# Siyou-Li/u2Tokenizer

Measured on NVIDIA H100. Metric: ct_volumes_per_sec, higher is better.
Workload: dtype bf16

## Files before the change

### include/u2b200.h

```cpp
#ifndef U2B200_H_
#define U2B200_H_

#include <stdint.h>

#if defined(__GNUC__)
#define U2_API __attribute__((visibility("default")))
#else
#define U2_API
#endif

#ifdef __cplusplus
extern "C" {
#endif

#define U2_OK 0
#define U2_ERR_ARG (-1)
#define U2_ERR_CUDA (-2)
#define U2_ERR_UNSUPPORTED (-3)

#define U2_DT_BF16 0
#define U2_DT_F32 1

#define U2_ACT_NONE 0
#define U2_ACT_GELU 1
#define U2_ACT_SILU 2

#define U2_EPI_NONE 0
#define U2_EPI_EXP_ROW 1
#define U2_EPI_DS_ROW 2

U2_API int u2_version(void);
U2_API const char* u2_last_error(void);
U2_API int u2_device_sm_count(void);

typedef struct u2_gemm_desc {
  int32_t M, N, K;
  int32_t zi, zo;
  int32_t b_zi_div;
  int64_t lda, a_stride_zi, a_stride_zo;
  int64_t ldb, b_stride_zi, b_stride_zo;
  int64_t ldc, c_stride_zi, c_stride_zo;
  int32_t c_dtype;
  float alpha;
  const float* bias;
  int32_t act;
  const void* residual;
  int64_t ldr;
  int32_t res_row_mod;
  int32_t row_div, row_stride, row_off;
  int32_t block_n;
  int32_t a_mn, b_mn;
  int32_t epi_op;
  const float* rowvec;
  int64_t rv_stride_zi, rv_stride_zo;
  const void* mul;
} u2_gemm_desc;

U2_API int u2_gemm_bf16(const void* A, const void* B, void* C, const u2_gemm_desc* desc, void* stream);

U2_API int u2_layernorm_bf16(const void* x, const void* residual, const float* gamma, const float* beta,
                             void* y, void* sum_out, int64_t rows, int32_t E, int64_t ldx, int64_t ldr,
                             int64_t ldy, float eps, void* stream);
U2_API int u2_rmsnorm_bf16(const void* x, const void* residual, const float* gamma, void* y, void* sum_out,
                           int64_t rows, int32_t E, int64_t ldx, int64_t ldr, int64_t ldy, float eps,
                           void* stream);

typedef struct u2_softmax_desc {
  int64_t in_s0, in_s1, in_s2;
  int64_t out_s0, out_s1, out_s2;
  int32_t n0, H, S, n;
  float scale;
  const float* rel_bias;
  int32_t rel_max;
  int32_t causal, causal_off;
  int32_t zero_pad_to;
  int32_t window;
} u2_softmax_desc;
U2_API int u2_softmax_f32_bf16(const float* in, void* out, const u2_softmax_desc* desc, void* stream);

U2_API int u2_silu_mul_bf16(const void* gate_up, void* out, int64_t rows, int32_t I, int64_t ldg,
                            int64_t ldo, int32_t interleaved, void* stream);

U2_API int u2_patchify_f32_bf16(const float* vol, void* rows, int64_t frames, int32_t d0, int32_t d1,
                                int32_t d2, int32_t p0, int32_t p1, int32_t p2, void* stream);
U2_API int u2_patch_embed_f32_bf16(const float* vol, const void* W, const float* bias, const void* pos, void* out,
                                   int64_t frames, int32_t d0, int32_t d1, int32_t d2, int32_t p0, int32_t p1, int32_t p2,
                                   int32_t N, int64_t out_frame_rows, void* stream);
U2_API int u2_set_rows_bf16(void* dst, const void* vec, int64_t n_rows, int64_t row_stride, int64_t row_off,
                            int32_t E, void* stream);
U2_API int u2_vit_frame_rows_bf16(void* dst, const void* cls, int64_t frames, int32_t Sp, int32_t S, int32_t E,
                                  void* stream);
U2_API int u2_transpose_heads_bf16(const void* in, void* out, int32_t B, int32_t S, int32_t H, int32_t Dh,
                                   int64_t in_sb, int64_t in_ss, int64_t in_sh, int64_t out_sb,
                                   int64_t out_sh, int64_t ld_out, void* stream);
U2_API int u2_spp_pool_bf16(const void* x, void* out, int64_t frames, int32_t g0, int32_t g1, int32_t g2,
                            int32_t ps, int32_t E, int64_t in_frame_stride, int64_t in_off, int64_t ldx,
                            int32_t sequence, void* stream);
U2_API int u2_multiscale_pool_bf16(const void* x, void* out, const float* gate_w, float gate_bias,
                                   float* logits_ws, int32_t B, int32_t K, int32_t E, int32_t dynamic,
                                   void* stream);
U2_API int64_t u2_multiscale_pool_ws_elems(int32_t B, int32_t K);
U2_API int u2_embed_splice_bf16(const int64_t* ids, const void* table, const void* vis, void* out, int32_t B,
                                int32_t L, int32_t E, int32_t n_vis, int64_t vocab, void* stream);

U2_API int u2_temporal_attention_bf16(const void* qkv, void* out, int32_t B, int32_t C, int32_t N, int32_t H,
                                      int32_t dh, int64_t ld_qkv, int64_t ld_out, float scale,
                                      const float* rel_bias, int32_t rel_max, void* stream);

typedef struct u2_rope_desc {
  int64_t rows, ld;
  int32_t dh, n_q_heads, n_k_heads, n_v_heads;
  const float* q_norm_w;
  const float* k_norm_w;
  float eps;
  const float* inv_freq;
  int32_t pos0, pos_div, pos_mod;
  const int32_t* pos0_dev;
  void* k_cache;
  void* v_cache;
  int32_t Tmax, rows_per_batch;
  int32_t pos0_per_batch;
} u2_rope_desc;
U2_API int u2_rope_bf16(void* x, const u2_rope_desc* desc, void* stream);

U2_API int u2_decode_attention_bf16(const void* q, const void* k_cache, const void* v_cache, void* out,
                                    int32_t B, int32_t Hq, int32_t Hkv, int32_t dh, int32_t Tmax, int32_t T,
                                    const int32_t* T_dev, int64_t ldq, int64_t ldo, float scale, int32_t T_per_seq,
                                    const int32_t* kv_src, int64_t ld_kv_src, void* stream);
U2_API int u2_decode_attention_window_bf16(const void* q, const void* k_cache, const void* v_cache, void* out,
                                           int32_t B, int32_t Hq, int32_t Hkv, int32_t dh, int32_t Tmax, int32_t T,
                                           const int32_t* T_dev, int64_t ldq, int64_t ldo, float scale,
                                           int32_t T_per_seq, const int32_t* kv_src, int64_t ld_kv_src,
                                           int32_t window, void* stream);

typedef struct u2_gemv_desc {
  int32_t B, N, K;
  int64_t ldx, ldw, ldy, ldr;
  int32_t y_dtype;
  const void* residual;
  const float* norm_gamma;
  float norm_eps;
  int32_t silu_pair;
} u2_gemv_desc;
U2_API int u2_gemv_bf16(const void* x, const void* w, void* y, const u2_gemv_desc* desc, void* stream);
U2_API int u2_argmax_f32(const float* logits, int64_t* out, uint64_t* scratch, int32_t B, int32_t V, int64_t ld,
                         void* stream);

#define U2_DLIN_STREAMK128 0
#define U2_DLIN_TILES64 1
typedef struct u2_dlinear_desc {
  int32_t B, N, K;
  int64_t ldx, ldw, ldy, ldr, ldxg;
  int32_t y_dtype;
  float* ws;
  int32_t* counters;
  const float* ssq_in;
  float eps;
  const void* residual;
  int32_t silu_pair;
  const float* gamma_next;
  void* xg;
  float* ssq_out;
  float* ssq_zero;
  int32_t pdl;
  void* dbg;
  int64_t ws_elems;
  const int32_t* dep_flags;
  int32_t dep_shift;
  int32_t* out_flags;
  int32_t sched;
} u2_dlinear_desc;
U2_API int u2_dlinear_bf16(const void* x, const void* w, void* y, const u2_dlinear_desc* desc, void* stream);
U2_API int64_t u2_dlinear_ws_elems(int32_t N, int32_t K);
typedef struct u2_dlinear_next {
  int32_t pre_stages;
  int32_t lookahead_units;
  int32_t n;
  const void* w[2];
  int32_t N[2], K[2];
  int64_t ldw[2];
  int32_t units[2];
} u2_dlinear_next;
U2_API int u2_dlinear_multi_bf16(const void* const* x, const void* const* w, void* const* y,
                                 const u2_dlinear_desc* descs, int32_t n_ops, uint32_t* gridbar,
                                 const int32_t* step_dev, int32_t pdl, const u2_dlinear_next* next, void* stream);
U2_API int u2_decode_embed_bf16(const int64_t* ids, const void* table, const float* gamma, void* x, void* xg,
                                float* ssq, float* ssq_zero, int32_t* step_counter, int32_t B, int32_t E,
                                int64_t vocab, void* stream);

typedef struct u2_fused_decode_desc {
  int32_t B, Hq, Hkv, dh, Tmax, pos;
  const int32_t* pos_dev;
  int64_t ldq, ldo;
  const float* q_norm_w;
  const float* k_norm_w;
  float eps;
  const float* inv_freq;
  float scale;
  int32_t kv_splits;
  int32_t pdl;
  int32_t pos_per_seq;
  const int32_t* kv_src;
  int64_t ld_kv_src;
  int32_t window;
} u2_fused_decode_desc;
U2_API int u2_decode_attention_fused_bf16(const void* qkv, void* k_cache, void* v_cache, void* out,
                                          const u2_fused_decode_desc* desc, void* stream);

U2_API int u2_topk_rows_f32(const float* scores, int64_t* out_idx, int32_t rows, int32_t T, int32_t K, int64_t ld,
                            int64_t idx_offset_per_row, void* stream);

typedef struct u2_fa_desc {
  int32_t B, H, Sq, Sk, dh;
  float scale;
  int64_t q_sb, q_ss, q_sh;
  int64_t k_sb, k_ss, k_sh;
  int64_t v_sb, v_ss, v_sh;
  int64_t out_sb, out_ss;
  float* lse;
} u2_fa_desc;
U2_API int u2_flash_attention_d64_bf16(const void* q, const void* k, const void* v, void* out, const u2_fa_desc* desc,
                                       void* stream);

U2_API int u2_sample_f32(const float* logits, int64_t* out, int32_t B, int32_t V, int64_t ld, float temperature,
                         int32_t top_k, float top_p, uint64_t seed, const int32_t* step_dev, int32_t step,
                         void* stream);

typedef struct u2_sample_params {
  float temperature;
  int32_t top_k;
  float top_p;
  int32_t reserved;
  uint64_t seed;
} u2_sample_params;
U2_API int u2_sample_dev_f32(const float* logits, int64_t* out, int32_t B, int32_t V, int64_t ld,
                             const u2_sample_params* params_dev, const int32_t* step_dev, int32_t step, void* stream);

#define U2_LP_MAX_EOS 8
#define U2_LP_MAX_BAD_WORDS 256
#define U2_LP_MAX_BAD_TOKENS 2048
typedef struct u2_logits_proc_params {
  float penalty;
  float inv_penalty;
  int32_t ngram;
  int32_t min_new;
  int32_t n_eos;
  int32_t n_bad;
  int32_t eos[U2_LP_MAX_EOS];
  int32_t bad_off[U2_LP_MAX_BAD_WORDS + 1];
  int32_t bad_tok[U2_LP_MAX_BAD_TOKENS];
} u2_logits_proc_params;
U2_API int u2_logits_process_f32(float* logits, int32_t B, int32_t V, int64_t ld, const int64_t* ids, int32_t* hist,
                                 int64_t ld_hist, int32_t hist_cap, const u2_logits_proc_params* params_dev,
                                 const int32_t* step_dev, int32_t step, void* stream);

#define U2_BEAM_MAX_BEAMS 16
#define U2_BEAM_MAX_EOS 8
#define U2_BEAM_MAX_KEEP 144
typedef struct u2_beam_params {
  double length_penalty;
  int32_t num_beams;
  int32_t beams_to_keep;
  int32_t early_stopping;
  int32_t max_new_tokens;
  int32_t n_eos;
  int32_t reserved;
  int32_t eos[U2_BEAM_MAX_EOS];
} u2_beam_params;
typedef struct u2_beam_step_desc {
  const u2_beam_params* params;
  int32_t prompts, V;
  const float* cand_val;
  const int32_t* cand_tok;
  float* running;
  float* fin_score;
  int32_t* fin_info;
  int32_t* flags;
  int64_t* ids;
  int32_t* rec;
  int64_t ld_rec;
  int32_t rec_rows;
  int32_t* kv_src;
  int64_t ld_kv_src;
  const int32_t* pos_dev;
  int32_t* hist;
  int64_t ld_hist;
  int32_t hist_cap;
  const int32_t* step_dev;
} u2_beam_step_desc;
U2_API int u2_log_softmax_f32(const float* x, float* y, int32_t rows, int32_t V, int64_t ldx, int64_t ldy, void* stream);
U2_API int u2_beam_topk_f32(const float* logprobs, int64_t ld, int32_t rows, int32_t V, const float* running,
                            const int32_t* flags, const u2_beam_params* params_dev, float* cand_val, int32_t* cand_tok,
                            void* stream);
U2_API int u2_beam_step(const u2_beam_step_desc* desc, int32_t step, void* stream);

typedef struct u2_logprob_desc {
  int32_t R, V, E;
  int64_t ldh, ldw;
  const int64_t* labels;
  void* ws;
  int64_t ws_bytes;
  float* lse;
  float* logit_sum;
  float* nll_acc;
} u2_logprob_desc;
U2_API int64_t u2_logprob_ws_bytes(int32_t R, int32_t V);
U2_API int u2_lmhead_logprob_bf16(const void* hidden, const void* W, float* logp, const u2_logprob_desc* desc,
                                  void* stream);

#define U2_PP_OK 0
#define U2_PP_EMPTY_FOREGROUND 1
#define U2_PP_DEGENERATE_SHAPE 2
#define U2_PP_FLAT_INTENSITY 3
typedef struct u2_preprocess_info {
  double a_min, a_max;
  int32_t lo[3], hi[3];
  int32_t out[3];
  float sigma[3];
  int32_t tail[3];
  int32_t status;
} u2_preprocess_info;
typedef struct u2_preprocess_desc {
  int32_t D, H, W;
  int32_t target, pad_depth;
  double lower_pct, upper_pct;
  void* ws;
  int64_t ws_bytes;
} u2_preprocess_desc;
U2_API int64_t u2_preprocess_ws_bytes(int32_t D, int32_t H, int32_t W);
U2_API int u2_preprocess_volume_f32(const float* vol, float* out, u2_preprocess_info* info,
                                    const u2_preprocess_desc* desc, void* stream);

#ifdef __cplusplus
}
#endif
#endif
```

### u2tokenizer_b200/_lib.py

```python
from __future__ import annotations

import ctypes as C
from pathlib import Path

_LIB_PATH = Path(__file__).resolve().parent / "libu2b200.so"
_lib = None


class GemmDesc(C.Structure):
    _fields_ = [
        ("M", C.c_int32), ("N", C.c_int32), ("K", C.c_int32),
        ("zi", C.c_int32), ("zo", C.c_int32), ("b_zi_div", C.c_int32),
        ("lda", C.c_int64), ("a_stride_zi", C.c_int64), ("a_stride_zo", C.c_int64),
        ("ldb", C.c_int64), ("b_stride_zi", C.c_int64), ("b_stride_zo", C.c_int64),
        ("ldc", C.c_int64), ("c_stride_zi", C.c_int64), ("c_stride_zo", C.c_int64),
        ("c_dtype", C.c_int32), ("alpha", C.c_float),
        ("bias", C.c_void_p),
        ("act", C.c_int32),
        ("residual", C.c_void_p),
        ("ldr", C.c_int64),
        ("res_row_mod", C.c_int32),
        ("row_div", C.c_int32), ("row_stride", C.c_int32), ("row_off", C.c_int32),
        ("block_n", C.c_int32),
        ("a_mn", C.c_int32), ("b_mn", C.c_int32),
        ("epi_op", C.c_int32),
        ("rowvec", C.c_void_p),
        ("rv_stride_zi", C.c_int64), ("rv_stride_zo", C.c_int64),
        ("mul", C.c_void_p),
    ]


class SoftmaxDesc(C.Structure):
    _fields_ = [
        ("in_s0", C.c_int64), ("in_s1", C.c_int64), ("in_s2", C.c_int64),
        ("out_s0", C.c_int64), ("out_s1", C.c_int64), ("out_s2", C.c_int64),
        ("n0", C.c_int32), ("H", C.c_int32), ("S", C.c_int32), ("n", C.c_int32),
        ("scale", C.c_float),
        ("rel_bias", C.c_void_p),
        ("rel_max", C.c_int32),
        ("causal", C.c_int32), ("causal_off", C.c_int32),
        ("zero_pad_to", C.c_int32),
        ("window", C.c_int32),
    ]


class RopeDesc(C.Structure):
    _fields_ = [
        ("rows", C.c_int64), ("ld", C.c_int64),
        ("dh", C.c_int32), ("n_q_heads", C.c_int32), ("n_k_heads", C.c_int32), ("n_v_heads", C.c_int32),
        ("q_norm_w", C.c_void_p), ("k_norm_w", C.c_void_p),
        ("eps", C.c_float),
        ("inv_freq", C.c_void_p),
        ("pos0", C.c_int32), ("pos_div", C.c_int32), ("pos_mod", C.c_int32),
        ("pos0_dev", C.c_void_p),
        ("k_cache", C.c_void_p), ("v_cache", C.c_void_p),
        ("Tmax", C.c_int32), ("rows_per_batch", C.c_int32),
        ("pos0_per_batch", C.c_int32),
    ]


class GemvDesc(C.Structure):
    _fields_ = [
        ("B", C.c_int32), ("N", C.c_int32), ("K", C.c_int32),
        ("ldx", C.c_int64), ("ldw", C.c_int64), ("ldy", C.c_int64), ("ldr", C.c_int64),
        ("y_dtype", C.c_int32),
        ("residual", C.c_void_p),
        ("norm_gamma", C.c_void_p),
        ("norm_eps", C.c_float),
        ("silu_pair", C.c_int32),
    ]


class DlinearDesc(C.Structure):
    _fields_ = [
        ("B", C.c_int32), ("N", C.c_int32), ("K", C.c_int32),
        ("ldx", C.c_int64), ("ldw", C.c_int64), ("ldy", C.c_int64), ("ldr", C.c_int64), ("ldxg", C.c_int64),
        ("y_dtype", C.c_int32),
        ("ws", C.c_void_p), ("counters", C.c_void_p),
        ("ssq_in", C.c_void_p),
        ("eps", C.c_float),
        ("residual", C.c_void_p),
        ("silu_pair", C.c_int32),
        ("gamma_next", C.c_void_p),
        ("xg", C.c_void_p),
        ("ssq_out", C.c_void_p),
        ("ssq_zero", C.c_void_p),
        ("pdl", C.c_int32),
        ("dbg", C.c_void_p),
        ("ws_elems", C.c_int64),
        ("dep_flags", C.c_void_p), ("dep_shift", C.c_int32), ("out_flags", C.c_void_p),
        ("sched", C.c_int32),
    ]


class FusedDecodeDesc(C.Structure):
    _fields_ = [
        ("B", C.c_int32), ("Hq", C.c_int32), ("Hkv", C.c_int32), ("dh", C.c_int32), ("Tmax", C.c_int32),
        ("pos", C.c_int32),
        ("pos_dev", C.c_void_p),
        ("ldq", C.c_int64), ("ldo", C.c_int64),
        ("q_norm_w", C.c_void_p), ("k_norm_w", C.c_void_p),
        ("eps", C.c_float),
        ("inv_freq", C.c_void_p),
        ("scale", C.c_float),
        ("kv_splits", C.c_int32), ("pdl", C.c_int32),
        ("pos_per_seq", C.c_int32),
        ("kv_src", C.c_void_p), ("ld_kv_src", C.c_int64),
        ("window", C.c_int32),
    ]


class DlinearNext(C.Structure):
    _fields_ = [
        ("pre_stages", C.c_int32), ("lookahead_units", C.c_int32), ("n", C.c_int32),
        ("w", C.c_void_p * 2),
        ("N", C.c_int32 * 2), ("K", C.c_int32 * 2),
        ("ldw", C.c_int64 * 2),
        ("units", C.c_int32 * 2),
    ]


class FaDesc(C.Structure):
    _fields_ = [
        ("B", C.c_int32), ("H", C.c_int32), ("Sq", C.c_int32), ("Sk", C.c_int32), ("dh", C.c_int32),
        ("scale", C.c_float),
        ("q_sb", C.c_int64), ("q_ss", C.c_int64), ("q_sh", C.c_int64),
        ("k_sb", C.c_int64), ("k_ss", C.c_int64), ("k_sh", C.c_int64),
        ("v_sb", C.c_int64), ("v_ss", C.c_int64), ("v_sh", C.c_int64),
        ("out_sb", C.c_int64), ("out_ss", C.c_int64),
        ("lse", C.c_void_p),
    ]


class LogprobDesc(C.Structure):
    _fields_ = [
        ("R", C.c_int32), ("V", C.c_int32), ("E", C.c_int32),
        ("ldh", C.c_int64), ("ldw", C.c_int64),
        ("labels", C.c_void_p), ("ws", C.c_void_p), ("ws_bytes", C.c_int64),
        ("lse", C.c_void_p), ("logit_sum", C.c_void_p), ("nll_acc", C.c_void_p),
    ]


class PreprocessInfo(C.Structure):
    _fields_ = [
        ("a_min", C.c_double), ("a_max", C.c_double),
        ("lo", C.c_int32 * 3), ("hi", C.c_int32 * 3), ("out", C.c_int32 * 3),
        ("sigma", C.c_float * 3), ("tail", C.c_int32 * 3), ("status", C.c_int32),
    ]


class PreprocessDesc(C.Structure):
    _fields_ = [
        ("D", C.c_int32), ("H", C.c_int32), ("W", C.c_int32), ("target", C.c_int32), ("pad_depth", C.c_int32),
        ("lower_pct", C.c_double), ("upper_pct", C.c_double),
        ("ws", C.c_void_p), ("ws_bytes", C.c_int64),
    ]


class SoftmaxBwdDesc(C.Structure):
    _fields_ = [
        ("p_s0", C.c_int64), ("p_s1", C.c_int64), ("p_s2", C.c_int64),
        ("dp_s0", C.c_int64), ("dp_s1", C.c_int64), ("dp_s2", C.c_int64),
        ("ds_s0", C.c_int64), ("ds_s1", C.c_int64), ("ds_s2", C.c_int64),
        ("n0", C.c_int32), ("H", C.c_int32), ("S", C.c_int32), ("n", C.c_int32),
        ("zero_pad_to", C.c_int32),
    ]


class AdamWDesc(C.Structure):
    _fields_ = [
        ("lr", C.c_float), ("beta1", C.c_float), ("beta2", C.c_float), ("eps", C.c_float), ("weight_decay", C.c_float),
        ("step", C.c_int32),
        ("grad_scale", C.c_void_p),
        ("seed", C.c_uint64), ("index_offset", C.c_int64),
    ]


class LoraDesc(C.Structure):
    _fields_ = [
        ("M", C.c_int32), ("K", C.c_int32), ("r", C.c_int32), ("n_adapters", C.c_int32),
        ("ldx", C.c_int64), ("ldu", C.c_int64),
        ("scale", C.c_float), ("p", C.c_float),
        ("seed", C.c_uint64),
        ("stream", C.c_int32 * 3),
        ("accumulate", C.c_int32),
    ]


LP_MAX_EOS, LP_MAX_BAD_WORDS, LP_MAX_BAD_TOKENS = 8, 256, 2048


class LogitsProcParams(C.Structure):
    _fields_ = [
        ("penalty", C.c_float), ("inv_penalty", C.c_float), ("ngram", C.c_int32), ("min_new", C.c_int32),
        ("n_eos", C.c_int32), ("n_bad", C.c_int32),
        ("eos", C.c_int32 * LP_MAX_EOS),
        ("bad_off", C.c_int32 * (LP_MAX_BAD_WORDS + 1)),
        ("bad_tok", C.c_int32 * LP_MAX_BAD_TOKENS),
    ]


BEAM_MAX_BEAMS, BEAM_MAX_EOS, BEAM_MAX_KEEP = 16, 8, 144


class BeamParams(C.Structure):
    _fields_ = [
        ("length_penalty", C.c_double),
        ("num_beams", C.c_int32), ("beams_to_keep", C.c_int32), ("early_stopping", C.c_int32),
        ("max_new_tokens", C.c_int32), ("n_eos", C.c_int32), ("reserved", C.c_int32),
        ("eos", C.c_int32 * BEAM_MAX_EOS),
    ]


class BeamStepDesc(C.Structure):
    _fields_ = [
        ("params", C.c_void_p),
        ("prompts", C.c_int32), ("V", C.c_int32),
        ("cand_val", C.c_void_p), ("cand_tok", C.c_void_p),
        ("running", C.c_void_p), ("fin_score", C.c_void_p), ("fin_info", C.c_void_p), ("flags", C.c_void_p),
        ("ids", C.c_void_p),
        ("rec", C.c_void_p), ("ld_rec", C.c_int64), ("rec_rows", C.c_int32),
        ("kv_src", C.c_void_p), ("ld_kv_src", C.c_int64),
        ("pos_dev", C.c_void_p),
        ("hist", C.c_void_p), ("ld_hist", C.c_int64), ("hist_cap", C.c_int32),
        ("step_dev", C.c_void_p),
    ]


_P, _I, _L, _F = C.c_void_p, C.c_int32, C.c_int64, C.c_float
SIGNATURES = {
    "u2_version": (C.c_int, []),
    "u2_last_error": (C.c_char_p, []),
    "u2_device_sm_count": (C.c_int, []),
    "u2_gemm_bf16": (C.c_int, [_P, _P, _P, C.POINTER(GemmDesc), _P]),
    "u2_layernorm_bf16": (C.c_int, [_P, _P, _P, _P, _P, _P, _L, _I, _L, _L, _L, _F, _P]),
    "u2_rmsnorm_bf16": (C.c_int, [_P, _P, _P, _P, _P, _L, _I, _L, _L, _L, _F, _P]),
    "u2_softmax_f32_bf16": (C.c_int, [_P, _P, C.POINTER(SoftmaxDesc), _P]),
    "u2_silu_mul_bf16": (C.c_int, [_P, _P, _L, _I, _L, _L, _I, _P]),
    "u2_patchify_f32_bf16": (C.c_int, [_P, _P, _L, _I, _I, _I, _I, _I, _I, _P]),
    "u2_patch_embed_f32_bf16": (C.c_int, [_P, _P, _P, _P, _P, _L, _I, _I, _I, _I, _I, _I, _I, _L, _P]),
    "u2_set_rows_bf16": (C.c_int, [_P, _P, _L, _L, _L, _I, _P]),
    "u2_vit_frame_rows_bf16": (C.c_int, [_P, _P, _L, _I, _I, _I, _P]),
    "u2_transpose_heads_bf16": (C.c_int, [_P, _P, _I, _I, _I, _I, _L, _L, _L, _L, _L, _L, _P]),
    "u2_spp_pool_bf16": (C.c_int, [_P, _P, _L, _I, _I, _I, _I, _I, _L, _L, _L, _I, _P]),
    "u2_multiscale_pool_bf16": (C.c_int, [_P, _P, _P, _F, _P, _I, _I, _I, _I, _P]),
    "u2_multiscale_pool_ws_elems": (C.c_int64, [_I, _I]),
    "u2_embed_splice_bf16": (C.c_int, [_P, _P, _P, _P, _I, _I, _I, _I, _L, _P]),
    "u2_temporal_attention_bf16": (C.c_int, [_P, _P, _I, _I, _I, _I, _I, _L, _L, _F, _P, _I, _P]),
    "u2_rope_bf16": (C.c_int, [_P, C.POINTER(RopeDesc), _P]),
    "u2_decode_attention_bf16": (C.c_int, [_P, _P, _P, _P, _I, _I, _I, _I, _I, _I, _P, _L, _L, _F, _I, _P, _L, _P]),
    "u2_decode_attention_window_bf16": (C.c_int, [_P, _P, _P, _P, _I, _I, _I, _I, _I, _I, _P, _L, _L, _F, _I, _P, _L,
                                                  _I, _P]),
    "u2_gemv_bf16": (C.c_int, [_P, _P, _P, C.POINTER(GemvDesc), _P]),
    "u2_argmax_f32": (C.c_int, [_P, _P, _P, _I, _I, _L, _P]),
    "u2_dlinear_bf16": (C.c_int, [_P, _P, _P, C.POINTER(DlinearDesc), _P]),
    "u2_decode_attention_fused_bf16": (C.c_int, [_P, _P, _P, _P, C.POINTER(FusedDecodeDesc), _P]),
    "u2_decode_embed_bf16": (C.c_int, [_P, _P, _P, _P, _P, _P, _P, _P, _I, _I, _L, _P]),
    "u2_flash_attention_d64_bf16": (C.c_int, [_P, _P, _P, _P, C.POINTER(FaDesc), _P]),
    "u2_sample_f32": (C.c_int, [_P, _P, _I, _I, _L, _F, _I, _F, C.c_uint64, _P, _I, _P]),
    "u2_sample_dev_f32": (C.c_int, [_P, _P, _I, _I, _L, _P, _P, _I, _P]),
    "u2_logits_process_f32": (C.c_int, [_P, _I, _I, _L, _P, _P, _L, _I, _P, _P, _I, _P]),
    "u2_topk_rows_f32": (C.c_int, [_P, _P, _I, _I, _I, _L, _L, _P]),
    "u2_log_softmax_f32": (C.c_int, [_P, _P, _I, _I, _L, _L, _P]),
    "u2_beam_topk_f32": (C.c_int, [_P, _L, _I, _I, _P, _P, _P, _P, _P, _P]),
    "u2_beam_step": (C.c_int, [C.POINTER(BeamStepDesc), _I, _P]),
    "u2_dlinear_ws_elems": (C.c_int64, [_I, _I]),
    "u2_dlinear_multi_bf16": (C.c_int, [_P, _P, _P, _P, _I, _P, _P, _I, _P, _P]),
    "u2_preprocess_ws_bytes": (C.c_int64, [_I, _I, _I]),
    "u2_preprocess_volume_f32": (C.c_int, [_P, _P, _P, C.POINTER(PreprocessDesc), _P]),
    "u2_logprob_ws_bytes": (C.c_int64, [_I, _I]),
    "u2_lmhead_logprob_bf16": (C.c_int, [_P, _P, _P, C.POINTER(LogprobDesc), _P]),
    "u2_transpose_bf16": (C.c_int, [_P, _P, _I, _I, _L, _L, _I, _L, _L, _P]),
    "u2_colsum_bf16": (C.c_int, [_P, _P, _L, _L, _L, _P]),
    "u2_gelu_bf16": (C.c_int, [_P, _P, _L, _P]),
    "u2_gelu_bwd_bf16": (C.c_int, [_P, _P, _P, _L, _P]),
    "u2_silu_mul_bwd_bf16": (C.c_int, [_P, _P, _P, _L, _I, _L, _L, _P]),
    "u2_layernorm_bwd_bf16": (C.c_int, [_P, _P, _P, _P, _P, _P, _P, _L, _I, _L, _L, _L, _L, _F, _P]),
    "u2_rmsnorm_bwd_bf16": (C.c_int, [_P, _P, _P, _P, _P, _P, _L, _I, _L, _L, _L, _L, _F, _P]),
    "u2_softmax_bwd_bf16": (C.c_int, [_P, _P, _P, C.POINTER(SoftmaxBwdDesc), _P]),
    "u2_relbias_grad_bf16": (C.c_int, [_P, _P, _I, _I, _I, _I, _L, _L, _L, _I, _P]),
    "u2_rowdot_bf16": (C.c_int, [_P, _P, _P, _I, _I, _I, _I, _L, _L, _L, _L, _L, _L, _P]),
    "u2_temporal_attention_bwd_bf16": (C.c_int, [_P, _P, _P, _I, _I, _I, _I, _I, _L, _L, _L, _F, _P, _P, _I, _P]),
    "u2_rope_bwd_bf16": (C.c_int, [_P, _P, C.POINTER(RopeDesc), _P, _P, _P]),
    "u2_spp_pool_bwd_bf16": (C.c_int, [_P, _P, _L, _I, _I, _I, _I, _I, _L, _L, _L, _L, _I, _P]),
    "u2_multiscale_pool_bwd_bf16": (C.c_int, [_P, _P, _P, _P, _P, _P, _P, _I, _I, _I, _I, _P]),
    "u2_embed_scatter_add_bf16": (C.c_int, [_P, _P, _P, _P, _I, _I, _I, _I, _L, _P]),
    "u2_group_sum_bf16": (C.c_int, [_P, _P, _L, _I, _I, _I, _L, _L, _P]),
    "u2_ce_bwd_f32_bf16": (C.c_int, [_P, _P, _P, _P, _P, _L, _I, _L, _L, _P]),
    "u2_dpo_loss_f32": (C.c_int, [_P, _P, _P, _P, _P, _I, _I, _F, _P]),
    "u2_adamw_bf16": (C.c_int, [_P, _P, _P, _P, _P, _L, C.POINTER(AdamWDesc), _P]),
    "u2_adamw_bf16_mom16": (C.c_int, [_P, _P, _P, _P, _P, _L, C.POINTER(AdamWDesc), _P]),
    "u2_adamw_f32grad": (C.c_int, [_P, _P, _P, _P, _P, _P, _L, C.POINTER(AdamWDesc), _P]),
    "u2_sumsq_bf16": (C.c_int, [_P, _P, _L, _P]),
    "u2_sumsq_f32": (C.c_int, [_P, _P, _L, _P]),
    "u2_add_bf16": (C.c_int, [_P, _P, _L, _P]),
    "u2_cast_f32_bf16": (C.c_int, [_P, _P, _L, _P]),
    "u2_cast_bf16_f32": (C.c_int, [_P, _P, _L, _P]),
    "u2_lora_down_bf16": (C.c_int, [_P, _P, _P, C.POINTER(LoraDesc), _P]),
    "u2_lora_wgrad_bf16": (C.c_int, [_P, _P, _P, C.POINTER(LoraDesc), _P]),
    "u2_lora_dgrad_bf16": (C.c_int, [_P, _P, _P, C.POINTER(LoraDesc), _P]),
}


def lib_path() -> Path:
    return _LIB_PATH


def load():
    global _lib
    if _lib is not None:
        return _lib
    if not _LIB_PATH.exists():
        raise RuntimeError(
            f"{_LIB_PATH} is missing: build it with `python -m u2tokenizer_b200.build` "
            "(there is no CPU / PyTorch fallback for the hot path)")
    lib = C.CDLL(str(_LIB_PATH))
    for name, (res, args) in SIGNATURES.items():
        fn = getattr(lib, name)
        fn.restype = res
        fn.argtypes = args
    _lib = lib
    return lib


KERNELS_PER_CALL = {"u2_multiscale_pool_bf16": 3, "u2_argmax_f32": 2, "u2_lmhead_logprob_bf16": 2,
                    "u2_preprocess_volume_f32": 14, "u2_multiscale_pool_bwd_bf16": 2}
_launches = 0


def launches() -> int:
    return _launches


def add_launches(n: int) -> None:
    global _launches
    _launches += n


def check(rc: int, what: str) -> None:
    global _launches
    _launches += KERNELS_PER_CALL.get(what, 1)
    if rc != 0:
        msg = load().u2_last_error()
        raise RuntimeError(f"{what} failed (code {rc}): {msg.decode() if msg else '?'}")
```

### u2tokenizer_b200/csrc/dlinear_wgmma.cu

```cuda
#include <cuda_bf16.h>
#include <math.h>
#include <stdio.h>
#include <stdlib.h>

#include "host_util.h"
#include "ptx.cuh"
#include "u2b200.h"

namespace u2 {

constexpr int kDlN = 16;
constexpr int kDlK = 64;
constexpr int kDlBBytes = kDlN * kDlK * 2;
constexpr int kDlThreads = 384;
constexpr int kDlMmaWarp0 = 8;
constexpr int kDlAccLd = 20;

template <int kM>
struct DlCfg {
  static constexpr int kABytes = kM * kDlK * 2;
  static constexpr int kStageBytes = kABytes + kDlBBytes;
#ifndef U2_DL_STAGES128
#define U2_DL_STAGES128 10
#endif
  static constexpr int kStages = (kM == 128) ? U2_DL_STAGES128 : 18;
  static constexpr int kAccBytes = 2 * kM * kDlAccLd * 4;
  static constexpr int kSmem = kStages * kStageBytes + kAccBytes + 1024 + 512;
};

struct DlinArgs {
  int B, N, K;
  int num_tiles, kblocks;
  float* ws;
  int max_slots;
  int* counters;
  const float* ssq_in;
  float inv_norm_dim, eps;
  const __nv_bfloat16* residual;
  long long ldr;
  void* y;
  long long ldy;
  int y_dtype;
  int silu_pair;
  const float* gamma_next;
  __nv_bfloat16* xg;
  long long ldxg;
  float* ssq_out;
  float* ssq_part;
  int* ssq_ticket;
  float* ssq_zero;
  const int* dep_flags;
  int dep_shift;
  int* out_flags;
  unsigned long long* dbg;
};

constexpr int kDlMaxOps = 4;

struct DlinMulti {
  CUtensorMap tw[kDlMaxOps];
  CUtensorMap tx[kDlMaxOps];
  DlinArgs op[kDlMaxOps];
  int n_ops;
  unsigned int* gridbar;
  const int* step_dev;
  unsigned long long* dbg;
  CUtensorMap tnext[2];
  int next_tiles[2], next_kblocks[2], next_units[2];
  int n_next;
  int pre_stages;
  int lookahead_units;
};

#define U2_STAMP(op, i)                                                                  \
  do {                                                                                   \
    if (mp.dbg) {                                                                        \
      unsigned long long t__;                                                            \
      asm volatile("mov.u64 %0, %%globaltimer;" : "=l"(t__));                           \
      mp.dbg[(blockIdx.x * kDlMaxOps + (op)) * 8 + (i)] = t__;                           \
    }                                                                                    \
  } while (0)

__device__ __forceinline__ unsigned int ld_acquire_u32(const unsigned int* p) {
  unsigned int v;
  asm volatile("ld.acquire.gpu.global.u32 %0, [%1];" : "=r"(v) : "l"(p) : "memory");
  return v;
}

__device__ __forceinline__ float4 ld_relaxed_f4(const float4* p) {
  float4 v;
  asm volatile("ld.relaxed.gpu.global.v4.f32 {%0, %1, %2, %3}, [%4];"
               : "=f"(v.x), "=f"(v.y), "=f"(v.z), "=f"(v.w)
               : "l"(p)
               : "memory");
  return v;
}

__device__ __forceinline__ void grid_barrier_wait(const unsigned int* bar, unsigned int target) {
  unsigned int v, spins = 0;
  do {
    asm volatile("ld.relaxed.gpu.global.u32 %0, [%1];" : "=r"(v) : "l"(bar) : "memory");
    if (++spins == (1u << 24)) {
      printf("u2 dlinear: grid barrier timed out (CTA %d sees %u of %u arrivals): CTAs of the launch are not co-resident\n",
             (int)blockIdx.x, v, target);
      __trap();
    }
  } while (v < target);
  asm volatile("fence.acq_rel.gpu;" ::: "memory");
}

struct UnitIter {
  int tile, kb, kblocks, tile_step;
  int left;
  __device__ __forceinline__ void next() {
    if (++kb == kblocks) {
      kb = 0;
      tile += tile_step;
    }
    --left;
  }
  __device__ __forceinline__ int seg_len() const {
    const int r = kblocks - kb;
    return r < left ? r : left;
  }
};

__device__ __forceinline__ UnitIter make_iter(int num_tiles, int kblocks, bool tiles) {
  UnitIter it;
  it.kblocks = kblocks;
  if (tiles) {
    const int mine = (num_tiles > (int)blockIdx.x) ? (num_tiles - (int)blockIdx.x + (int)gridDim.x - 1) / (int)gridDim.x : 0;
    it.tile = blockIdx.x;
    it.kb = 0;
    it.tile_step = gridDim.x;
    it.left = mine * kblocks;
  } else {
    const long long units = (long long)num_tiles * kblocks;
    const long long G = units < (long long)gridDim.x ? units : (long long)gridDim.x;
    it.tile_step = 1;
    if ((long long)blockIdx.x >= G) {
      it.tile = 0;
      it.kb = 0;
      it.left = 0;
    } else {
      const long long base = units * blockIdx.x / G;
      const long long end = units * (blockIdx.x + 1) / G;
      it.tile = (int)(base / kblocks);
      it.kb = (int)(base - (long long)it.tile * kblocks);
      it.left = (int)(end - base);
    }
  }
  return it;
}

__device__ __forceinline__ void wait_tile_flag(const int* flags, int t, int step, unsigned char* ready, int tag) {
  if (ready[t] == (unsigned char)tag) return;
  const int t4 = t & ~3;
  for (;;) {
    int4 f;
    asm volatile("ld.relaxed.gpu.global.v4.s32 {%0, %1, %2, %3}, [%4];"
                 : "=r"(f.x), "=r"(f.y), "=r"(f.z), "=r"(f.w)
                 : "l"(flags + t4)
                 : "memory");
    if (f.x >= step) ready[t4] = (unsigned char)tag;
    if (f.y >= step) ready[t4 + 1] = (unsigned char)tag;
    if (f.z >= step) ready[t4 + 2] = (unsigned char)tag;
    if (f.w >= step) ready[t4 + 3] = (unsigned char)tag;
    if (ready[t] == (unsigned char)tag) break;
  }
  asm volatile("fence.acq_rel.gpu;" ::: "memory");
  asm volatile("fence.proxy.async;" ::: "memory");
}

template <int kM>
__global__ void __launch_bounds__(kDlThreads, 1)
dlinear_wgmma_kernel(const __grid_constant__ DlinMulti mp) {
  using Cfg = DlCfg<kM>;
  constexpr int kStages = Cfg::kStages;
  constexpr int kABytes = Cfg::kABytes;
  constexpr int kStageBytes = Cfg::kStageBytes;
  constexpr bool kTiles = (kM == 64);
  extern __shared__ uint8_t smem_raw[];
  uint8_t* smem = reinterpret_cast<uint8_t*>((reinterpret_cast<uintptr_t>(smem_raw) + 1023) & ~static_cast<uintptr_t>(1023));
  uint8_t* smem_a = smem;
  uint8_t* smem_b = smem + kStages * kABytes;
  float* smem_acc = reinterpret_cast<float*>(smem + kStages * kStageBytes);
  uint64_t* bars = reinterpret_cast<uint64_t*>(smem + kStages * kStageBytes + Cfg::kAccBytes);
  uint64_t* full_bar = bars;
  uint64_t* empty_bar = bars + kStages;
  uint64_t* acc_full_bar = bars + 2 * kStages;
  uint64_t* acc_empty_bar = bars + 2 * kStages + 2;
  __shared__ unsigned char s_ready[1024];
  if (threadIdx.x < 256) reinterpret_cast<unsigned int*>(s_ready)[threadIdx.x] = 0u;

  const int warp_idx = threadIdx.x / 32;
  const int lane = threadIdx.x % 32;
  const int n_ops = mp.n_ops;

  if (warp_idx == 0 && lane == 0) {
    for (int i = 0; i < n_ops; ++i) {
      tma_prefetch_desc(&mp.tw[i]);
      tma_prefetch_desc(&mp.tx[i]);
    }
  }
  if (warp_idx == 1 && lane == 0) {
    for (int s = 0; s < kStages; ++s) {
      mbar_init(&full_bar[s], 1);
      mbar_init(&empty_bar[s], 4);
    }
    for (int s = 0; s < 2; ++s) {
      mbar_init(&acc_full_bar[s], 4);
      mbar_init(&acc_empty_bar[s], 4);
    }
    fence_barrier_init();
  }
  __syncthreads();
  asm volatile("griddepcontrol.launch_dependents;" ::: "memory");

  if (warp_idx == 0) {
    if (lane == 0) {
      const uint64_t pol_w = l2_policy_evict_first();
      int stage = 0;
      uint32_t phase = 0;
      unsigned int target = 0;
      int step = 0;
      for (int oi = 0; oi < n_ops; ++oi) {
        const DlinArgs& p = mp.op[oi];
        UnitIter it = make_iter(p.num_tiles, p.kblocks, kTiles);
        const int pre_cap = (oi == 0 || mp.pre_stages <= 0 || mp.pre_stages > kStages) ? kStages : mp.pre_stages;
        const int npre = it.left < pre_cap ? it.left : pre_cap;
        int st = stage;
        uint32_t ph = phase;
        UnitIter pre = it;
        for (int j = 0; j < npre; ++j) {
          mbar_wait(&empty_bar[st], ph ^ 1);
          mbar_arrive_expect_tx(&full_bar[st], kStageBytes);
          tma_load_4d_hint(smem_a + st * kABytes, &mp.tw[oi], &full_bar[st], pre.kb * kDlK, pre.tile * kM, 0, 0, pol_w);
          pre.next();
          if (++st == kStages) {
            st = 0;
            ph ^= 1;
          }
        }
        {
          UnitIter la = pre;
          for (int j = 0; j < mp.lookahead_units && la.left > 0; ++j) {
            tma_prefetch_l2_4d(&mp.tw[oi], la.kb * kDlK, la.tile * kM, 0, 0);
            la.next();
          }
        }
        U2_STAMP(oi, 0);
        if (oi == 0) {
          asm volatile("griddepcontrol.wait;" ::: "memory");
          step = *reinterpret_cast<const volatile int*>(mp.step_dev);
          target = (unsigned int)step * gridDim.x;
        } else if (!p.dep_flags) {
          grid_barrier_wait(mp.gridbar + (oi - 1), target);
          asm volatile("fence.proxy.async;" ::: "memory");
        }
        U2_STAMP(oi, 1);
        for (int j = 0; j < npre; ++j) {
          if (oi > 0 && p.dep_flags) wait_tile_flag(p.dep_flags, it.kb >> p.dep_shift, step, s_ready, oi);
          tma_load_4d(smem_b + stage * kDlBBytes, &mp.tx[oi], &full_bar[stage], it.kb * kDlK, 0, 0, 0);
          it.next();
          if (++stage == kStages) {
            stage = 0;
            phase ^= 1;
          }
        }
        while (it.left > 0) {
          mbar_wait(&empty_bar[stage], phase ^ 1);
          mbar_arrive_expect_tx(&full_bar[stage], kStageBytes);
          tma_load_4d_hint(smem_a + stage * kABytes, &mp.tw[oi], &full_bar[stage], it.kb * kDlK, it.tile * kM, 0, 0, pol_w);
          if (oi > 0 && p.dep_flags) wait_tile_flag(p.dep_flags, it.kb >> p.dep_shift, step, s_ready, oi);
          tma_load_4d(smem_b + stage * kDlBBytes, &mp.tx[oi], &full_bar[stage], it.kb * kDlK, 0, 0, 0);
          it.next();
          if (++stage == kStages) {
            stage = 0;
            phase ^= 1;
          }
        }
      }
      for (int jn = 0; jn < mp.n_next; ++jn) {
        UnitIter la = make_iter(mp.next_tiles[jn], mp.next_kblocks[jn], kTiles);
        for (int j = 0; j < mp.next_units[jn] && la.left > 0; ++j) {
          tma_prefetch_l2_4d(&mp.tnext[jn], la.kb * kDlK, la.tile * kM, 0, 0);
          la.next();
        }
      }
    }
  } else if (warp_idx >= kDlMmaWarp0) {
    const int w = warp_idx - kDlMmaWarp0;
    int stage = 0;
    uint32_t phase = 0;
    int acc = 0;
    uint32_t acc_phase = 0;
    for (int oi = 0; oi < n_ops; ++oi) {
      UnitIter it = make_iter(mp.op[oi].num_tiles, mp.op[oi].kblocks, kTiles);
      bool first_unit = true;
      while (it.left > 0) {
        const int seg = it.seg_len();
        float d[kM / 64][8];
        for (int j = 0; j < seg; ++j) {
          mbar_wait(&full_bar[stage], phase);
          if (first_unit) {
            if (threadIdx.x == kDlMmaWarp0 * 32) U2_STAMP(oi, 2);
            first_unit = false;
          }
          const uint64_t a_desc = gmma_desc_sw128(smem_u32(smem_a + stage * kABytes));
          const uint64_t b_desc = gmma_desc_sw128(smem_u32(smem_b + stage * kDlBBytes));
          wgmma_fence();
#pragma unroll
          for (int k = 0; k < kDlK / 16; ++k) {
#pragma unroll
            for (int mh = 0; mh < kM / 64; ++mh)
              wgmma_m64n16k16_ss(d[mh], a_desc + 512 * mh + 2 * k, b_desc + 2 * k, (j == 0 && k == 0) ? 0u : 1u);
          }
          wgmma_commit();
          wgmma_wait<0>();
          if (lane == 0) mbar_arrive(&empty_bar[stage]);
          it.next();
          if (++stage == kStages) {
            stage = 0;
            phase ^= 1;
          }
        }
        mbar_wait(&acc_empty_bar[acc], acc_phase ^ 1);
        float* dst = smem_acc + acc * (kM * kDlAccLd);
#pragma unroll
        for (int mh = 0; mh < kM / 64; ++mh) {
#pragma unroll
          for (int e = 0; e < 8; ++e) {
            const int r = mh * 64 + w * 16 + (lane >> 2) + 8 * ((e >> 1) & 1);
            dst[r * kDlAccLd + 8 * (e >> 2) + 2 * (lane & 3) + (e & 1)] = d[mh][e];
          }
        }
        __syncwarp();
        if (lane == 0) mbar_arrive(&acc_full_bar[acc]);
        if (it.left == 0 && threadIdx.x == kDlMmaWarp0 * 32) U2_STAMP(oi, 3);
        if (++acc == 2) {
          acc = 0;
          acc_phase ^= 1;
        }
      }
    }
  } else if (warp_idx >= 4) {
    const int q = warp_idx - 4;
    const int et = threadIdx.x - 128;
    const int trow = (kM == 128) ? et : (q * 16 + (lane & 15));
    const bool tvalid = (kM == 128) ? true : (lane < 16);
    asm volatile("griddepcontrol.wait;" ::: "memory");
    const unsigned int target = (unsigned int)(*reinterpret_cast<const volatile int*>(mp.step_dev)) * gridDim.x;
    int acc = 0;
    uint32_t acc_phase = 0;
    for (int oi = 0; oi < n_ops; ++oi) {
      const DlinArgs& p = mp.op[oi];
      UnitIter it = make_iter(p.num_tiles, p.kblocks, kTiles);
      bool prev_done = (oi == 0);
      if (oi > 0 && !p.dep_flags) {
        if (et == 0) grid_barrier_wait(mp.gridbar + (oi - 1), target);
        asm volatile("bar.sync 1, 128;" ::: "memory");
        prev_done = true;
      }
      while (it.left > 0) {
        const int tile = it.tile;
        const int seg_kb = it.seg_len();
        it.left -= seg_kb;
        it.kb += seg_kb;
        if (it.kb == it.kblocks) {
          it.kb = 0;
          it.tile += it.tile_step;
        }

        const int row = tile * kM + trow;
        const bool whole = (seg_kb == p.kblocks);
        int gf = (int)blockIdx.x, n_contrib = 0;
        if (!whole) {
          const long long units = (long long)p.num_tiles * p.kblocks;
          const long long G = units < (long long)gridDim.x ? units : (long long)gridDim.x;
          const long long u0 = (long long)tile * p.kblocks;
          gf = (int)(((u0 + 1) * G + units - 1) / units) - 1;
          n_contrib = (int)(((u0 + p.kblocks) * G + units - 1) / units) - 1 - gf;
        }
        const bool finalizer = (gf == (int)blockIdx.x);
        const int nvec = (p.B + 3) >> 2;
        const bool row_ok = tvalid && row < p.N;
        unsigned short res_raw[16];
        float rs[16];
        float gam = 0.f;
        if (finalizer) {
          if (!prev_done) {
            if (et == 0) grid_barrier_wait(mp.gridbar + (oi - 1), target);
            asm volatile("bar.sync 1, 128;" ::: "memory");
            prev_done = true;
          }
#pragma unroll
          for (int b = 0; b < 16; ++b) {
            res_raw[b] = 0;
            rs[b] = 1.f;
            if (b < p.B) {
              if (p.residual && !p.silu_pair && row_ok)
                res_raw[b] = __ldcg(reinterpret_cast<const unsigned short*>(p.residual) + (long long)b * p.ldr + row);
              if (p.ssq_in) rs[b] = __ldcg(p.ssq_in + b);
            }
          }
          if (p.gamma_next && row_ok) gam = __ldg(p.gamma_next + row);
        }

        mbar_wait(&acc_full_bar[acc], acc_phase);
        if (et == 0 && it.left == 0) U2_STAMP(oi, 4);
        uint32_t v[16];
        {
          const uint32_t src = smem_u32(smem_acc + acc * (kM * kDlAccLd) + trow * kDlAccLd);
#pragma unroll
          for (int c = 0; c < 4; ++c) {
            const uint4 x = lds128(src + 16 * c);
            v[4 * c] = x.x; v[4 * c + 1] = x.y; v[4 * c + 2] = x.z; v[4 * c + 3] = x.w;
          }
        }
        __syncwarp();
        if ((threadIdx.x & 31) == 0) mbar_arrive(&acc_empty_bar[acc]);
        if (++acc == 2) {
          acc = 0;
          acc_phase ^= 1;
        }

        float f[16];
#pragma unroll
        for (int b = 0; b < 16; ++b) f[b] = __uint_as_float(v[b]);
        if (!finalizer) {
          const int slot = (int)blockIdx.x - gf - 1;
          float4* dst = reinterpret_cast<float4*>(p.ws + (((long long)tile * p.max_slots + slot) * kM + trow) * kDlN);
          if (tvalid) {
#pragma unroll
            for (int c = 0; c < 4; ++c)
              if (c < nvec) __stcg(dst + c, make_float4(f[4 * c], f[4 * c + 1], f[4 * c + 2], f[4 * c + 3]));
          }
        } else {
          if (et == 0) U2_STAMP(oi, 6);
          if (n_contrib > 0 && tvalid) {
            const long long slot_stride = (long long)kM * kDlN / 4;
            float4* src0 = reinterpret_cast<float4*>(p.ws + (((long long)tile * p.max_slots) * kM + trow) * kDlN);
            const float4 sent = make_float4(__uint_as_float(0xffffffffu), __uint_as_float(0xffffffffu),
                                            __uint_as_float(0xffffffffu), __uint_as_float(0xffffffffu));
#pragma unroll
            for (int c = 0; c < 4; ++c) {
              if (c >= nvec) break;
              constexpr int kMaxSlots = 8;
              for (int s0 = 0; s0 < n_contrib; s0 += kMaxSlots) {
                float4 t[kMaxSlots];
                bool ok;
                unsigned int spins = 0;
                do {
                  ok = true;
#pragma unroll
                  for (int sl = 0; sl < kMaxSlots; ++sl)
                    if (s0 + sl < n_contrib) t[sl] = ld_relaxed_f4(src0 + (s0 + sl) * slot_stride + c);
#pragma unroll
                  for (int sl = 0; sl < kMaxSlots; ++sl)
                    if (s0 + sl < n_contrib) {
                      ok = ok && (__float_as_uint(t[sl].x) != 0xffffffffu) && (__float_as_uint(t[sl].y) != 0xffffffffu) &&
                           (__float_as_uint(t[sl].z) != 0xffffffffu) && (__float_as_uint(t[sl].w) != 0xffffffffu);
                    }
                } while (!ok && ++spins < (1u << 22));
#pragma unroll
                for (int sl = 0; sl < kMaxSlots; ++sl)
                  if (s0 + sl < n_contrib) {
                    f[4 * c] += t[sl].x; f[4 * c + 1] += t[sl].y; f[4 * c + 2] += t[sl].z; f[4 * c + 3] += t[sl].w;
                    __stcg(src0 + (s0 + sl) * slot_stride + c, sent);
                  }
              }
            }
          }
          if (et == 0) U2_STAMP(oi, 7);
          if (p.ssq_zero && tile == 0 && et < 16) p.ssq_zero[et] = 0.f;
          float sq[16];
#pragma unroll
          for (int b = 0; b < 16; ++b) {
            sq[b] = 0.f;
            if (b < p.B) {
              float val = f[b];
              if (p.ssq_in) val *= rsqrtf(rs[b] * p.inv_norm_dim + p.eps);
              if (p.silu_pair) {
                const float me = __bfloat162float(__float2bfloat16(val));
                const float other = __shfl_down_sync(0xffffffffu, me, 1);
                if (row_ok && (trow & 1) == 0) {
                  const float o = __fdividef(me, 1.f + __expf(-me)) * other;
                  reinterpret_cast<__nv_bfloat16*>(p.y)[(long long)b * p.ldy + (row >> 1)] = __float2bfloat16(o);
                }
              } else if (row_ok) {
                val += __bfloat162float(__ushort_as_bfloat16(res_raw[b]));
                if (p.y_dtype == U2_DT_BF16) {
                  const __nv_bfloat16 o = __float2bfloat16(val);
                  reinterpret_cast<__nv_bfloat16*>(p.y)[(long long)b * p.ldy + row] = o;
                  val = __bfloat162float(o);
                } else {
                  reinterpret_cast<float*>(p.y)[(long long)b * p.ldy + row] = val;
                }
                if (p.gamma_next) p.xg[(long long)b * p.ldxg + row] = __float2bfloat16(val * gam);
                sq[b] = val * val;
              }
            }
          }
          if (p.ssq_out) {
            __shared__ float s_sq[4][16];
            __shared__ int s_last;
#pragma unroll
            for (int b = 0; b < 16; ++b) {
              float s = sq[b];
#pragma unroll
              for (int o = 16; o > 0; o >>= 1) s += __shfl_xor_sync(0xffffffffu, s, o);
              if (lane == 0) s_sq[q][b] = s;
            }
            asm volatile("bar.sync 1, 128;" ::: "memory");
            if (et < 16) {
              __stcg(p.ssq_part + (long long)tile * 16 + et, ((s_sq[0][et] + s_sq[1][et]) + s_sq[2][et]) + s_sq[3][et]);
              __threadfence();
            }
            asm volatile("bar.sync 1, 128;" ::: "memory");
            if (et == 0) s_last = (atomicAdd(p.ssq_ticket, 1) == p.num_tiles - 1);
            asm volatile("bar.sync 1, 128;" ::: "memory");
            if (s_last) {
              __shared__ float s_grp[8][16];
              __threadfence();
              const int col = et & 15, grp = et >> 4;
              float t = 0.f;
              for (int i0 = grp; i0 < p.num_tiles; i0 += 32) {
                float v[4];
#pragma unroll
                for (int u = 0; u < 4; ++u) {
                  const int i = i0 + 8 * u;
                  v[u] = (i < p.num_tiles) ? __ldcg(p.ssq_part + (long long)i * 16 + col) : 0.f;
                }
#pragma unroll
                for (int u = 0; u < 4; ++u) {
                  const int i = i0 + 8 * u;
                  if (i < p.num_tiles) {
                    t += v[u];
                    __stcg(p.ssq_part + (long long)i * 16 + col, __uint_as_float(0xffffffffu));
                  }
                }
              }
              s_grp[grp][col] = t;
              asm volatile("bar.sync 1, 128;" ::: "memory");
              if (et < p.B) {
                float tot = 0.f;
#pragma unroll
                for (int g = 0; g < 8; ++g) tot += s_grp[g][et];
                p.ssq_out[et] += tot;
              }
              if (et == 0) *p.ssq_ticket = 0;
            }
          }
          if (p.out_flags) {
            asm volatile("bar.sync 1, 128;" ::: "memory");
            if (et == 0) {
              const int stepv = (int)(target / gridDim.x);
              asm volatile("st.release.gpu.global.s32 [%0], %1;" ::"l"(p.out_flags + tile), "r"(stepv) : "memory");
            }
          }
        }
      }
      if (et == 0) U2_STAMP(oi, 5);
      if (oi + 1 < n_ops) {
        asm volatile("bar.sync 1, 128;" ::: "memory");
        if (et == 0) asm volatile("red.release.gpu.global.add.u32 [%0], 1;" ::"l"(mp.gridbar + oi) : "memory");
      }
    }
  }
}

__global__ void __launch_bounds__(256)
decode_embed_kernel(const long long* __restrict__ ids, const __nv_bfloat16* __restrict__ table,
                    const float* __restrict__ gamma, __nv_bfloat16* __restrict__ x, __nv_bfloat16* __restrict__ xg,
                    float* __restrict__ ssq, float* __restrict__ ssq_zero, int* __restrict__ step_counter, int E,
                    long long vocab) {
  const int b = blockIdx.x;
  if (b == 0 && threadIdx.x == 0 && step_counter) *step_counter += 1;
  long long id = ids[b];
  if (id < 0) id = 0;
  if (id >= vocab) id = vocab - 1;
  const __nv_bfloat16* src = table + id * E;
  float s = 0.f;
  for (int i = threadIdx.x; i < E; i += blockDim.x) {
    const __nv_bfloat16 v = src[i];
    const float f = __bfloat162float(v);
    x[(long long)b * E + i] = v;
    xg[(long long)b * E + i] = __float2bfloat16(f * gamma[i]);
    s += f * f;
  }
  __shared__ float red[8];
#pragma unroll
  for (int o = 16; o > 0; o >>= 1) s += __shfl_xor_sync(0xffffffffu, s, o);
  if ((threadIdx.x & 31) == 0) red[threadIdx.x >> 5] = s;
  __syncthreads();
  if (threadIdx.x == 0) {
    float t = 0.f;
    for (int w = 0; w < (int)(blockDim.x >> 5); ++w) t += red[w];
    ssq[b] = t;
    if (ssq_zero) ssq_zero[b] = 0.f;
  }
}

}

using namespace u2;

static int fill_op(const void* x, const void* w, void* y, const u2_dlinear_desc* d, DlinArgs* p, CUtensorMap* tw,
                   CUtensorMap* tx, int kM) {
  if (!x || !w || !y || !d || !d->ws || !d->counters) return set_error(U2_ERR_ARG, "dlinear: null pointer");
  if (d->B < 1 || d->B > kDlN) return set_error(U2_ERR_UNSUPPORTED, "dlinear: 1 <= B <= 16 (got %d)", d->B);
  if (d->N <= 0 || d->K <= 0 || (d->K % kDlK)) return set_error(U2_ERR_ARG, "dlinear: K must be a positive multiple of 64");
  if ((d->ldx & 7) || (d->ldw & 7)) return set_error(U2_ERR_ARG, "dlinear: ldx/ldw must be multiples of 8");
  if (d->silu_pair && (d->N & 1)) return set_error(U2_ERR_ARG, "dlinear: silu_pair needs an even N");
  if (d->gamma_next && !d->xg) return set_error(U2_ERR_ARG, "dlinear: gamma_next needs xg");
  p->B = d->B; p->N = d->N; p->K = d->K;
  p->num_tiles = (d->N + kM - 1) / kM;
  p->kblocks = d->K / kDlK;
  p->ws = d->ws; p->counters = d->counters;
  p->max_slots = 1;
  if (kM == 128) {
    const long long units = (long long)p->num_tiles * p->kblocks;
    int g = num_sms();
    if (g <= 0) g = 132;
    long long rmin = units / g;
    if (rmin < 1) rmin = 1;
    const long long cmax = (p->kblocks + rmin - 1) / rmin + 1;
    p->max_slots = (int)cmax;
    if ((long long)p->num_tiles * cmax * kM * kDlN > d->ws_elems)
      return set_error(U2_ERR_ARG, "dlinear: workspace too small (%lld fp32 needed for N=%d K=%d)",
                       (long long)p->num_tiles * cmax * kM * kDlN, d->N, d->K);
  }
  p->ssq_in = d->ssq_in;
  p->inv_norm_dim = 1.0f / (float)d->K;
  p->eps = d->eps;
  p->residual = reinterpret_cast<const __nv_bfloat16*>(d->residual);
  p->ldr = d->ldr;
  p->y = y; p->ldy = d->ldy; p->y_dtype = d->y_dtype;
  p->silu_pair = d->silu_pair;
  p->gamma_next = d->gamma_next;
  p->xg = reinterpret_cast<__nv_bfloat16*>(d->xg);
  p->ldxg = d->ldxg;
  p->ssq_out = d->ssq_out;
  p->ssq_part = nullptr;
  p->ssq_ticket = nullptr;
  if (d->ssq_out) {
    const long long slots = (kM == 128) ? (long long)p->num_tiles * p->max_slots * kM * kDlN : 0;
    if (slots + (long long)p->num_tiles * kDlN > d->ws_elems)
      return set_error(U2_ERR_ARG, "dlinear: workspace too small for the sums of squares (%lld fp32 needed for N=%d K=%d)",
                       slots + (long long)p->num_tiles * kDlN, d->N, d->K);
    p->ssq_part = d->ws + slots;
    p->ssq_ticket = d->counters + (d->N + 63) / 64;
  }
  p->ssq_zero = d->ssq_zero;
  p->dep_flags = d->dep_flags;
  p->dep_shift = d->dep_shift;
  p->out_flags = d->out_flags;
  p->dbg = nullptr;
  int rc = make_tmap_bf16_4d(tw, w, d->K, d->N, 1, 1, d->ldw, 0, 0, kDlK, kM);
  if (rc) return rc;
  return make_tmap_bf16_4d(tx, x, d->K, d->B, 1, 1, d->ldx, 0, 0, kDlK, kDlN);
}

template <int kM>
static int launch_multi_t(DlinMulti& mp, int pdl, cudaStream_t stream) {
  static bool configured = false;
  if (!configured) {
    cudaError_t e = cudaFuncSetAttribute(dlinear_wgmma_kernel<kM>, cudaFuncAttributeMaxDynamicSharedMemorySize, DlCfg<kM>::kSmem);
    if (e != cudaSuccess) return set_error(U2_ERR_CUDA, "dlinear: cudaFuncSetAttribute: %s", cudaGetErrorString(e));
    int per_sm = 0;
    e = cudaOccupancyMaxActiveBlocksPerMultiprocessor(&per_sm, dlinear_wgmma_kernel<kM>, kDlThreads, DlCfg<kM>::kSmem);
    if (e != cudaSuccess || per_sm < 1)
      return set_error(U2_ERR_CUDA, "dlinear: kernel cannot be resident on an SM (%s, %d CTA/SM): set U2_MULTI_OP=0",
                       cudaGetErrorString(e), per_sm);
    configured = true;
  }
  int grid = num_sms();
  if (grid <= 0) return set_error(U2_ERR_CUDA, "dlinear: cannot query SM count");
  if (mp.n_ops == 1) {
    const long long work = (kM == 64) ? mp.op[0].num_tiles : (long long)mp.op[0].num_tiles * mp.op[0].kblocks;
    if (work < grid) grid = (int)work;
  }
  cudaLaunchConfig_t cfg = {};
  cfg.gridDim = dim3((unsigned)grid);
  cfg.blockDim = dim3(kDlThreads);
  cfg.dynamicSmemBytes = DlCfg<kM>::kSmem;
  cfg.stream = stream;
  cudaLaunchAttribute attr[1];
  attr[0].id = cudaLaunchAttributeProgrammaticStreamSerialization;
  attr[0].val.programmaticStreamSerializationAllowed = 1;
  cfg.attrs = attr;
  cfg.numAttrs = pdl ? 1 : 0;
  cudaError_t e = cudaLaunchKernelEx(&cfg, dlinear_wgmma_kernel<kM>, mp);
  if (e != cudaSuccess) return set_error(U2_ERR_CUDA, "dlinear launch: %s", cudaGetErrorString(e));
  return U2_OK;
}

static int launch_multi(DlinMulti& mp, int kM, int pdl, cudaStream_t stream) {
  return kM == 64 ? launch_multi_t<64>(mp, pdl, stream) : launch_multi_t<128>(mp, pdl, stream);
}

static inline int tile_m_of(const u2_dlinear_desc* d) { return d->sched == U2_DLIN_TILES64 ? 64 : 128; }


extern "C" U2_API int64_t u2_dlinear_ws_elems(int32_t N, int32_t K) {
  if (N <= 0 || K <= 0) return 0;
  const long long tiles = (N + 127) / 128, kblocks = (K + kDlK - 1) / kDlK;
  int g = num_sms();
  if (g <= 0) g = 132;
  long long rmin = tiles * kblocks / g;
  if (rmin < 1) rmin = 1;
  const long long cmax = (kblocks + rmin - 1) / rmin + 1;
  return tiles * cmax * 128 * kDlN + (N + 63) / 64 * kDlN;
}

extern "C" U2_API int u2_dlinear_bf16(const void* x, const void* w, void* y, const u2_dlinear_desc* d, void* stream) {
  static DlinMulti mp;
  mp.n_ops = 1;
  if (!d) return set_error(U2_ERR_ARG, "dlinear: null descriptor");
  const int kM = tile_m_of(d);
  int rc = fill_op(x, w, y, d, &mp.op[0], &mp.tw[0], &mp.tx[0], kM);
  if (rc) return rc;
  mp.gridbar = nullptr;
  mp.n_next = 0;
  mp.lookahead_units = 0;
  mp.pre_stages = 0;
  mp.dbg = reinterpret_cast<unsigned long long*>(d->dbg);
  mp.step_dev = d->counters;
  return launch_multi(mp, kM, d->pdl, reinterpret_cast<cudaStream_t>(stream));
}

extern "C" U2_API int u2_dlinear_multi_bf16(const void* const* x, const void* const* w, void* const* y,
                                            const u2_dlinear_desc* descs, int32_t n_ops, uint32_t* gridbar,
                                            const int32_t* step_dev, int32_t pdl, const u2_dlinear_next* next,
                                            void* stream) {
  if (!x || !w || !y || !descs) return set_error(U2_ERR_ARG, "dlinear_multi: null pointer");
  if (n_ops < 1 || n_ops > kDlMaxOps) return set_error(U2_ERR_ARG, "dlinear_multi: 1 <= n_ops <= %d", kDlMaxOps);
  if (n_ops > 1 && (!gridbar || !step_dev)) return set_error(U2_ERR_ARG, "dlinear_multi: gridbar / step_dev required");
  static DlinMulti mp;
  mp.n_ops = n_ops;
  const int kM = tile_m_of(&descs[0]);
  for (int i = 0; i < n_ops; ++i) {
    if (tile_m_of(&descs[i]) != kM) return set_error(U2_ERR_ARG, "dlinear_multi: all ops of a launch must share one schedule");
    int rc = fill_op(x[i], w[i], y[i], &descs[i], &mp.op[i], &mp.tw[i], &mp.tx[i], kM);
    if (rc) return rc;
  }
  mp.gridbar = gridbar;
  mp.lookahead_units = next ? next->lookahead_units : 0;
  mp.pre_stages = next ? next->pre_stages : 0;
  mp.n_next = 0;
  if (next) {
    for (int j = 0; j < 2 && j < next->n; ++j) {
      if (!next->w[j] || next->K[j] % kDlK || next->N[j] <= 0) return set_error(U2_ERR_ARG, "dlinear_multi: bad look-ahead weight");
      int rc = make_tmap_bf16_4d(&mp.tnext[j], next->w[j], next->K[j], next->N[j], 1, 1, next->ldw[j], 0, 0, kDlK, kM);
      if (rc) return rc;
      mp.next_tiles[j] = (next->N[j] + kM - 1) / kM;
      mp.next_kblocks[j] = next->K[j] / kDlK;
      mp.next_units[j] = next->units[j];
      mp.n_next = j + 1;
    }
  }
  mp.dbg = reinterpret_cast<unsigned long long*>(descs[0].dbg);
  mp.step_dev = step_dev ? step_dev : descs[0].counters;
  return launch_multi(mp, kM, pdl, reinterpret_cast<cudaStream_t>(stream));
}

extern "C" U2_API int u2_decode_embed_bf16(const int64_t* ids, const void* table, const float* gamma, void* x,
                                           void* xg, float* ssq, float* ssq_zero, int32_t* step_counter, int32_t B,
                                           int32_t E, int64_t vocab, void* stream) {
  if (!ids || !table || !gamma || !x || !xg || !ssq) return set_error(U2_ERR_ARG, "decode_embed: null pointer");
  if (B < 1 || B > kDlN) return set_error(U2_ERR_UNSUPPORTED, "decode_embed: 1 <= B <= 16");
  decode_embed_kernel<<<B, 256, 0, reinterpret_cast<cudaStream_t>(stream)>>>(
      reinterpret_cast<const long long*>(ids), reinterpret_cast<const __nv_bfloat16*>(table), gamma,
      reinterpret_cast<__nv_bfloat16*>(x), reinterpret_cast<__nv_bfloat16*>(xg), ssq, ssq_zero, step_counter, E, vocab);
  U2_CHECK_LAUNCH("decode_embed");
  return U2_OK;
}
```

### u2tokenizer_b200/csrc/ptx.cuh

```cuda
#pragma once
#include <cuda_runtime.h>
#include <cuda.h>
#include <stdint.h>

namespace u2 {

__device__ __forceinline__ uint32_t smem_u32(const void* p) {
  return static_cast<uint32_t>(__cvta_generic_to_shared(p));
}

__device__ __forceinline__ uint32_t lane_id() {
  uint32_t l;
  asm volatile("mov.u32 %0, %%laneid;" : "=r"(l));
  return l;
}

__device__ __forceinline__ void mbar_init(uint64_t* bar, uint32_t count) {
  asm volatile("mbarrier.init.shared::cta.b64 [%0], %1;" ::"r"(smem_u32(bar)), "r"(count));
}

__device__ __forceinline__ void fence_barrier_init() {
  asm volatile("fence.mbarrier_init.release.cluster;" ::: "memory");
}

__device__ __forceinline__ void mbar_arrive(uint64_t* bar) {
  asm volatile("mbarrier.arrive.shared::cta.b64 _, [%0];" ::"r"(smem_u32(bar)) : "memory");
}

__device__ __forceinline__ void mbar_arrive_expect_tx(uint64_t* bar, uint32_t bytes) {
  asm volatile("mbarrier.arrive.expect_tx.shared::cta.b64 _, [%0], %1;" ::"r"(smem_u32(bar)),
               "r"(bytes)
               : "memory");
}

__device__ __forceinline__ bool mbar_try_wait(uint64_t* bar, uint32_t parity) {
  uint32_t ok;
  asm volatile(
      "{\n\t"
      ".reg .pred p;\n\t"
      "mbarrier.try_wait.parity.shared::cta.b64 p, [%1], %2;\n\t"
      "selp.u32 %0, 1, 0, p;\n\t"
      "}"
      : "=r"(ok)
      : "r"(smem_u32(bar)), "r"(parity)
      : "memory");
  return ok != 0;
}

__device__ __forceinline__ void mbar_wait(uint64_t* bar, uint32_t parity) {
  while (!mbar_try_wait(bar, parity)) {
  }
}

__device__ __forceinline__ void tma_prefetch_desc(const CUtensorMap* m) {
  asm volatile("prefetch.tensormap [%0];" ::"l"(reinterpret_cast<uint64_t>(m)) : "memory");
}

__device__ __forceinline__ void tma_load_4d(void* smem_dst, const CUtensorMap* m, uint64_t* bar,
                                            int c0, int c1, int c2, int c3) {
  asm volatile(
      "cp.async.bulk.tensor.4d.shared::cluster.global.tile.mbarrier::complete_tx::bytes "
      "[%0], [%1, {%3, %4, %5, %6}], [%2];"
      :
      : "r"(smem_u32(smem_dst)), "l"(reinterpret_cast<uint64_t>(m)), "r"(smem_u32(bar)), "r"(c0),
        "r"(c1), "r"(c2), "r"(c3)
      : "memory");
}

__device__ __forceinline__ void tma_store_4d(const CUtensorMap* m, uint32_t smem_src, int c0, int c1, int c2, int c3) {
  asm volatile("cp.async.bulk.tensor.4d.global.shared::cta.bulk_group [%0, {%2, %3, %4, %5}], [%1];"
               :
               : "l"(reinterpret_cast<uint64_t>(m)), "r"(smem_src), "r"(c0), "r"(c1), "r"(c2), "r"(c3)
               : "memory");
}
__device__ __forceinline__ void bulk_commit_group() { asm volatile("cp.async.bulk.commit_group;" ::: "memory"); }
template <int kPending>
__device__ __forceinline__ void bulk_wait_group_read() {
  asm volatile("cp.async.bulk.wait_group.read %0;" ::"n"(kPending) : "memory");
}
template <int kPending>
__device__ __forceinline__ void bulk_wait_group() {
  asm volatile("cp.async.bulk.wait_group %0;" ::"n"(kPending) : "memory");
}

__device__ __forceinline__ void tma_prefetch_l2_4d(const CUtensorMap* m, int c0, int c1, int c2, int c3) {
  asm volatile("cp.async.bulk.prefetch.tensor.4d.L2.global.tile [%0, {%1, %2, %3, %4}];"
               :
               : "l"(reinterpret_cast<uint64_t>(m)), "r"(c0), "r"(c1), "r"(c2), "r"(c3)
               : "memory");
}

__device__ __forceinline__ uint64_t l2_policy_evict_first() {
  uint64_t p;
  asm volatile("createpolicy.fractional.L2::evict_first.b64 %0, 1.0;" : "=l"(p));
  return p;
}

__device__ __forceinline__ void tma_load_4d_hint(void* smem_dst, const CUtensorMap* m, uint64_t* bar, int c0, int c1,
                                                 int c2, int c3, uint64_t policy) {
  asm volatile(
      "cp.async.bulk.tensor.4d.shared::cluster.global.tile.mbarrier::complete_tx::bytes.L2::cache_hint "
      "[%0], [%1, {%3, %4, %5, %6}], [%2], %7;"
      :
      : "r"(smem_u32(smem_dst)), "l"(reinterpret_cast<uint64_t>(m)), "r"(smem_u32(bar)), "r"(c0),
        "r"(c1), "r"(c2), "r"(c3), "l"(policy)
      : "memory");
}

__device__ __forceinline__ void tma_load_3d(void* smem_dst, const CUtensorMap* m, uint64_t* bar,
                                            int c0, int c1, int c2) {
  asm volatile(
      "cp.async.bulk.tensor.3d.shared::cluster.global.tile.mbarrier::complete_tx::bytes "
      "[%0], [%1, {%3, %4, %5}], [%2];"
      :
      : "r"(smem_u32(smem_dst)), "l"(reinterpret_cast<uint64_t>(m)), "r"(smem_u32(bar)), "r"(c0),
        "r"(c1), "r"(c2)
      : "memory");
}

__device__ __forceinline__ float4 lds128_f32(uint32_t addr) {
  float4 v;
  asm volatile("ld.shared.v4.f32 {%0, %1, %2, %3}, [%4];" : "=f"(v.x), "=f"(v.y), "=f"(v.z), "=f"(v.w) : "r"(addr));
  return v;
}
__device__ __forceinline__ uint4 lds128(uint32_t addr) {
  uint4 v;
  asm volatile("ld.shared.v4.b32 {%0, %1, %2, %3}, [%4];" : "=r"(v.x), "=r"(v.y), "=r"(v.z), "=r"(v.w) : "r"(addr));
  return v;
}
__device__ __forceinline__ void sts128(uint32_t addr, const uint4& v) {
  asm volatile("st.shared.v4.b32 [%0], {%1, %2, %3, %4};" ::"r"(addr), "r"(v.x), "r"(v.y), "r"(v.z), "r"(v.w) : "memory");
}

__device__ __forceinline__ void sts64(uint32_t addr, uint32_t lo, uint32_t hi) {
  asm volatile("st.shared.v2.b32 [%0], {%1, %2};" ::"r"(addr), "r"(lo), "r"(hi) : "memory");
}

__device__ __forceinline__ void fence_proxy_async_smem() {
  asm volatile("fence.proxy.async.shared::cta;" ::: "memory");
}

__device__ __forceinline__ void wgmma_fence() { asm volatile("wgmma.fence.sync.aligned;" ::: "memory"); }
__device__ __forceinline__ void wgmma_commit() { asm volatile("wgmma.commit_group.sync.aligned;" ::: "memory"); }
template <int kPending>
__device__ __forceinline__ void wgmma_wait() {
  asm volatile("wgmma.wait_group.sync.aligned %0;" ::"n"(kPending) : "memory");
}

__device__ __forceinline__ uint64_t gmma_desc_sw128(uint32_t smem_addr, uint32_t lbo_bytes = 16) {
  uint64_t d = 0;
  d |= static_cast<uint64_t>((smem_addr & 0x3FFFFu) >> 4);
  d |= static_cast<uint64_t>(lbo_bytes >> 4) << 16;
  d |= static_cast<uint64_t>(1024u >> 4) << 32;
  d |= static_cast<uint64_t>(1) << 62;
  return d;
}

template <int kTransA, int kTransB>
__device__ __forceinline__ void wgmma_m64n64k16_ss(float (&d)[32], uint64_t a_desc, uint64_t b_desc, uint32_t accumulate) {
  asm volatile(
      "{\n\t"
      ".reg .pred p;\n\t"
      "setp.ne.b32 p, %34, 0;\n\t"
      "wgmma.mma_async.sync.aligned.m64n64k16.f32.bf16.bf16 "
      "{%0, %1, %2, %3, %4, %5, %6, %7, %8, %9, %10, %11, %12, %13, %14, %15, %16, %17, %18, %19, %20, %21, %22, %23, %24, %25, %26, %27, %28, %29, %30, %31}, %32, %33, p, 1, 1, %35, %36;\n\t"
      "}"
      : "+f"(d[0]), "+f"(d[1]), "+f"(d[2]), "+f"(d[3]), "+f"(d[4]), "+f"(d[5]), "+f"(d[6]), "+f"(d[7]), "+f"(d[8]), "+f"(d[9]), "+f"(d[10]), "+f"(d[11]), "+f"(d[12]), "+f"(d[13]), "+f"(d[14]), "+f"(d[15]), "+f"(d[16]), "+f"(d[17]), "+f"(d[18]), "+f"(d[19]), "+f"(d[20]), "+f"(d[21]), "+f"(d[22]), "+f"(d[23]), "+f"(d[24]), "+f"(d[25]), "+f"(d[26]), "+f"(d[27]), "+f"(d[28]), "+f"(d[29]), "+f"(d[30]), "+f"(d[31])
      : "l"(a_desc), "l"(b_desc), "r"(accumulate), "n"(kTransA), "n"(kTransB));
}

template <int kTransB>
__device__ __forceinline__ void wgmma_m64n64k16_rs(float (&d)[32], const uint32_t (&a)[4], uint64_t b_desc) {
  asm volatile(
      "{\n\t"
      "wgmma.mma_async.sync.aligned.m64n64k16.f32.bf16.bf16 "
      "{%0, %1, %2, %3, %4, %5, %6, %7, %8, %9, %10, %11, %12, %13, %14, %15, %16, %17, %18, %19, %20, %21, %22, %23, %24, %25, %26, %27, %28, %29, %30, %31}, {%32, %33, %34, %35}, %36, 1, 1, 1, %37;\n\t"
      "}"
      : "+f"(d[0]), "+f"(d[1]), "+f"(d[2]), "+f"(d[3]), "+f"(d[4]), "+f"(d[5]), "+f"(d[6]), "+f"(d[7]), "+f"(d[8]), "+f"(d[9]), "+f"(d[10]), "+f"(d[11]), "+f"(d[12]), "+f"(d[13]), "+f"(d[14]), "+f"(d[15]), "+f"(d[16]), "+f"(d[17]), "+f"(d[18]), "+f"(d[19]), "+f"(d[20]), "+f"(d[21]), "+f"(d[22]), "+f"(d[23]), "+f"(d[24]), "+f"(d[25]), "+f"(d[26]), "+f"(d[27]), "+f"(d[28]), "+f"(d[29]), "+f"(d[30]), "+f"(d[31])
      : "r"(a[0]), "r"(a[1]), "r"(a[2]), "r"(a[3]), "l"(b_desc), "n"(kTransB));
}

__device__ __forceinline__ void wgmma_m64n16k16_ss(float (&d)[8], uint64_t a_desc, uint64_t b_desc, uint32_t accumulate) {
  asm volatile(
      "{\n\t"
      ".reg .pred p;\n\t"
      "setp.ne.b32 p, %10, 0;\n\t"
      "wgmma.mma_async.sync.aligned.m64n16k16.f32.bf16.bf16 "
      "{%0, %1, %2, %3, %4, %5, %6, %7}, %8, %9, p, 1, 1, 0, 0;\n\t"
      "}"
      : "+f"(d[0]), "+f"(d[1]), "+f"(d[2]), "+f"(d[3]), "+f"(d[4]), "+f"(d[5]), "+f"(d[6]), "+f"(d[7])
      : "l"(a_desc), "l"(b_desc), "r"(accumulate));
}


}
```

### u2tokenizer_b200/engine.py

```python
from __future__ import annotations

import math
from dataclasses import dataclass
from typing import Dict, List, Optional, Tuple

import torch

from . import _lib, ops
from .geometry import Geometry

BF16, F32 = torch.bfloat16, torch.float32
REL_MAX = 512


def _pad8(n: int) -> int:
    return (n + 7) // 8 * 8


@dataclass(frozen=True)
class LogitsProcessors:
    repetition_penalty: float = 1.0
    no_repeat_ngram_size: int = 0
    min_new_tokens: int = 0
    eos_token_ids: Tuple[int, ...] = ()
    bad_words_ids: Tuple[Tuple[int, ...], ...] = ()

    def neutral(self) -> bool:
        return (self.repetition_penalty == 1.0 and self.no_repeat_ngram_size == 0 and not self.bad_words_ids
                and (self.min_new_tokens == 0 or not self.eos_token_ids))


@dataclass(frozen=True)
class BeamSearch:
    num_beams: int
    length_penalty: float = 1.0
    early_stopping: object = False
    num_return_sequences: int = 1
    pad_token_id: Optional[int] = None


class _Take:

    def __init__(self, sd: Dict[str, torch.Tensor], device):
        self.sd, self.dev = sd, device

    def has(self, k):
        return k in self.sd

    def bf(self, k) -> torch.Tensor:
        return self.sd.pop(k).to(device=self.dev, dtype=BF16).contiguous()

    def f32(self, k) -> torch.Tensor:
        return self.sd.pop(k).to(device=self.dev, dtype=BF16).to(F32).contiguous()

    def cat_bf(self, keys) -> torch.Tensor:
        return torch.cat([self.bf(k) for k in keys], dim=0).contiguous()

    def cat_f32(self, keys) -> torch.Tensor:
        return torch.cat([self.f32(k) for k in keys], dim=0).contiguous()


@dataclass
class _SelfAttnW:
    wqkv: torch.Tensor
    bqkv: torch.Tensor
    wd: torch.Tensor
    bd: torch.Tensor
    rel: Optional[torch.Tensor]
    seq_first: bool = False


@dataclass
class _CrossAttnW:
    wq: torch.Tensor
    bq: torch.Tensor
    wkv: torch.Tensor
    bkv: torch.Tensor
    wd: Optional[torch.Tensor]
    bd: Optional[torch.Tensor]


class U2Engine:
    def __init__(self, geom: Geometry, state_dict: Dict[str, torch.Tensor], device="cuda",
                 attn_workspace_bytes: int = 6 << 30, decode_impl: str = "tcgen05"):
        if not torch.cuda.is_available():
            raise RuntimeError("U2Engine needs a CUDA device: the hot path has no CPU implementation")
        from . import _lib
        _lib.load()
        self.g = geom
        self.dev = torch.device(device)
        self.attn_ws = attn_workspace_bytes
        self.decode_impl = decode_impl
        import os
        from . import _lib
        self.num_sms = int(_lib.load().u2_device_sm_count())
        self.fwd_graph = os.environ.get("U2_FWD_GRAPH", "1") != "0"
        self.attn_pdl = os.environ.get("U2_ATTN_PDL", "0") != "0"
        self.pdl = os.environ.get("U2_PDL", "1") != "0"
        self.multi_op = os.environ.get("U2_MULTI_OP", "1") != "0"
        self.fused_patch_embed = os.environ.get("U2_FUSED_PATCH_EMBED", "0") != "0"
        self.use_flash = os.environ.get("U2_FLASH", "1") != "0"
        self.fine_deps = os.environ.get("U2_FINE_DEPS", "0") != "0"
        self.dl_sched = int(os.environ.get("U2_DL_SCHED", "0"))
        self.pre_stages = int(os.environ.get("U2_PRE_STAGES", "0"))
        self.l2_lookahead_units = int(os.environ.get("U2_L2_LOOKAHEAD", "0"))
        self.l2_next_units = int(os.environ.get("U2_L2_NEXT", "-1"))
        if geom.vision_select_feature != "patch":
            raise NotImplementedError("only vision_select_feature='patch' is supported (the spp projector needs it)")
        t = _Take(dict(state_dict), self.dev)
        self._prep_vit(t)
        self._prep_projector(t)
        if geom.enable_u2tokenizer:
            self._prep_tokenizer(t)
        self._prep_decoder(t)
        self._gen_state = None
        self._fwd_state = None
        self._sampling = None
        self._samp_dev = None
        self._samp_host = None
        self._procs = None
        self._lp_dev = None
        self._lp_host = None
        self._beam = None
        self._beam_dev = None
        self._beam_host = None
        self.last_beam_scores = None

    def _prep_vit(self, t: _Take):
        g = self.g
        v = "model.vision_tower.vision_tower."
        self.pe_w = t.bf(v + "patch_embedding.patch_embeddings.1.weight")
        self.pe_b = t.f32(v + "patch_embedding.patch_embeddings.1.bias")
        self.pos = t.bf(v + "patch_embedding.position_embeddings").view(g.n_patches, g.vit_hidden)
        self.cls = t.bf(v + "cls_token").view(g.vit_hidden)
        self.vit = []
        for i in range(g.vit_layers):
            b = f"{v}blocks.{i}."
            self.vit.append(dict(
                ln1g=t.f32(b + "norm1.weight"), ln1b=t.f32(b + "norm1.bias"),
                wqkv=t.bf(b + "attn.qkv.weight"),
                bqkv=t.f32(b + "attn.qkv.bias") if t.has(b + "attn.qkv.bias") else None,
                wo=t.bf(b + "attn.out_proj.weight"), bo=t.f32(b + "attn.out_proj.bias"),
                ln2g=t.f32(b + "norm2.weight"), ln2b=t.f32(b + "norm2.bias"),
                w1=t.bf(b + "mlp.linear1.weight"), b1=t.f32(b + "mlp.linear1.bias"),
                w2=t.bf(b + "mlp.linear2.weight"), b2=t.f32(b + "mlp.linear2.bias")))
        self.vit_ng = t.f32(v + "norm.weight")
        self.vit_nb = t.f32(v + "norm.bias")

    def _prep_projector(self, t: _Take):
        g = self.g
        p = "model.mm_projector.projector."
        self.proj = [(t.bf(p + "0.weight"), t.f32(p + "0.bias"))]
        for i in range(1, int(g.proj_layer_num)):
            idx = 2 * i if g.proj_layer_type == "mlp" else i
            self.proj.append((t.bf(p + f"{idx}.weight"), t.f32(p + f"{idx}.bias")))

    def _self_attn_w(self, t: _Take, pre: str) -> _SelfAttnW:
        if self.g.attn_type not in ("rma", "rope"):
            return _SelfAttnW(wqkv=t.bf(pre + "in_proj_weight"), bqkv=t.f32(pre + "in_proj_bias"),
                              wd=t.bf(pre + "out_proj.weight"), bd=t.f32(pre + "out_proj.bias"), rel=None,
                              seq_first=True)
        rel = t.f32(pre + "relative_bias") if self.g.attn_type == "rma" else None
        return _SelfAttnW(
            wqkv=t.cat_bf([pre + "wq.weight", pre + "wk.weight", pre + "wv.weight"]),
            bqkv=t.cat_f32([pre + "wq.bias", pre + "wk.bias", pre + "wv.bias"]),
            wd=t.bf(pre + "dense.weight"), bd=t.f32(pre + "dense.bias"), rel=rel)

    def _cross_attn_w(self, t: _Take, pre: str, compress: bool = False) -> _CrossAttnW:
        if compress:
            for k in ("wv.weight", "wv.bias", "dense.weight", "dense.bias"):
                t.sd.pop(pre + k, None)
            return _CrossAttnW(wq=t.bf(pre + "wq.weight"), bq=t.f32(pre + "wq.bias"),
                               wkv=t.bf(pre + "wk.weight"), bkv=t.f32(pre + "wk.bias"), wd=None, bd=None)
        return _CrossAttnW(wq=t.bf(pre + "wq.weight"), bq=t.f32(pre + "wq.bias"),
                           wkv=t.cat_bf([pre + "wk.weight", pre + "wv.weight"]),
                           bkv=t.cat_f32([pre + "wk.bias", pre + "wv.bias"]),
                           wd=t.bf(pre + "dense.weight"), bd=t.f32(pre + "dense.bias"))

    def _prep_tokenizer(self, t: _Take):
        g = self.g
        u = "model.u2tokenizer."
        self.queries = t.bf(u + "query_tokens").view(g.num_3d_query_token, g.hidden_size)
        self.svr = []
        for i in range(g.u2t_num_layers):
            l = f"{u}svt_module.attention_network.layers.{i}."
            self.svr.append((self._self_attn_w(t, l + "spatial_attention."),
                             self._self_attn_w(t, l + "temporal_attention.")))
        self.score_w = t.bf(u + "svt_module.token_selection.score_net.weight")
        self.score_b = t.f32(u + "svt_module.token_selection.score_net.bias")
        self.gate_w, self.gate_b = None, 0.0
        if g.enable_dmtp:
            self.gate_w = t.f32(u + "svt_module.dynamic_pool.gate_fc.weight").view(-1)
            self.gate_b = float(t.f32(u + "svt_module.dynamic_pool.gate_fc.bias").item())
        self.tta = []
        for i in range(g.u2t_num_layers):
            l = f"{u}tta_module.layers_vt.{i}."
            self.tta.append(dict(
                self_attn=self._self_attn_w(t, l + "self_attention."),
                vis=self._cross_attn_w(t, l + "visual_cross_attention."),
                txt=self._cross_attn_w(t, l + "text_cross_attention."),
                ns=(t.f32(l + "norm_self.weight"), t.f32(l + "norm_self.bias")),
                nv=(t.f32(l + "norm_cross_v.weight"), t.f32(l + "norm_cross_v.bias")),
                nt=(t.f32(l + "norm_cross_t.weight"), t.f32(l + "norm_cross_t.bias"))))
        self.linagg = self._cross_attn_w(t, u + "tta_module.layer_linagg.linear_aggregator.", compress=True)
        dh = g.hidden_size // g.u2t_num_heads
        self.u2t_inv_freq = (1.0 / (10000 ** (torch.arange(0, dh, 2, dtype=F32) / dh))).to(self.dev)

    def _prep_decoder(self, t: _Take):
        g = self.g
        self.embed = t.bf("model.embed_tokens.weight")
        self.layers = []
        phi3 = g.decoder_family == "phi3"
        for i in range(g.num_hidden_layers):
            l = f"model.layers.{i}."
            if phi3:
                wqkv = t.bf(l + "self_attn.qkv_proj.weight")
                gate, up = t.bf(l + "mlp.gate_up_proj.weight").chunk(2, dim=0)
            else:
                wqkv = t.cat_bf([l + "self_attn.q_proj.weight", l + "self_attn.k_proj.weight",
                                 l + "self_attn.v_proj.weight"])
                gate, up = t.bf(l + "mlp.gate_proj.weight"), t.bf(l + "mlp.up_proj.weight")
            self.layers.append(dict(
                ln1=t.f32(l + "input_layernorm.weight"),
                wqkv=wqkv,
                qn=t.f32(l + "self_attn.q_norm.weight") if g.qk_norm else None,
                kn=t.f32(l + "self_attn.k_norm.weight") if g.qk_norm else None,
                wo=t.bf(l + "self_attn.o_proj.weight"),
                ln2=t.f32(l + "post_attention_layernorm.weight"),
                wgu=torch.stack([gate, up], dim=1).view(2 * g.intermediate_size, g.hidden_size).contiguous(),
                wdown=t.bf(l + "mlp.down_proj.weight")))
            del gate, up
        self.final_norm = t.f32("model.norm.weight")
        self.lm_head = self.embed if (g.tie_word_embeddings or not t.has("lm_head.weight")) else t.bf("lm_head.weight")
        self.inv_freq = self._decoder_inv_freq().to(self.dev)

    def _decoder_inv_freq(self) -> torch.Tensor:
        g = self.g
        dh = g.head_dim
        inv = 1.0 / (g.rope_theta ** (torch.arange(0, dh, 2, dtype=F32) / dh))
        rs = g.rope_scaling
        if rs and rs.get("rope_type", rs.get("type")) == "llama3":
            factor, lo, hi = rs["factor"], rs["low_freq_factor"], rs["high_freq_factor"]
            old = rs["original_max_position_embeddings"]
            wavelen = 2 * math.pi / inv
            inv_l = torch.where(wavelen > old / lo, inv / factor, inv)
            smooth = (old / wavelen - lo) / (hi - lo)
            smoothed = (1 - smooth) * inv_l / factor + smooth * inv_l
            is_med = ~(wavelen < old / hi) & ~(wavelen > old / lo)
            inv = torch.where(is_med, smoothed, inv_l)
        elif rs:
            raise NotImplementedError(f"rope_scaling {rs} not supported")
        return inv

    def _attention(self, q: torch.Tensor, k: torch.Tensor, v: torch.Tensor, out: torch.Tensor, scale: float,
                   rel_bias: Optional[torch.Tensor] = None, causal: bool = False, window: int = 0):
        b, Sq, h, dh = q.shape
        Sk, hk = k.shape[1], k.shape[2]
        Skp = _pad8(Sk)
        if dh == 64 and h == hk and rel_bias is None and not causal and self.use_flash:
            return ops.flash_attention_d64(q, k, v, out, scale)
        per_b = h * Sq * Skp * 6
        chunk = max(1, min(b, self.attn_ws // max(per_b, 1)))
        dev = q.device
        sc = torch.empty(chunk, h, Sq, Skp, device=dev, dtype=F32)
        pr = torch.empty(chunk, h, Sq, Skp, device=dev, dtype=BF16)
        for b0 in range(0, b, chunk):
            nb = min(chunk, b - b0)
            qq, kk, vv, oo = q[b0:b0 + nb], k[b0:b0 + nb], v[b0:b0 + nb], out[b0:b0 + nb]
            ops.gemm(qq, kk, sc, M=Sq, N=Sk, K=dh, lda=qq.stride(1), ldb=kk.stride(1), ldc=Skp, zi=h, zo=nb,
                     b_zi_div=h // hk, a_strides=(qq.stride(2), qq.stride(0)), b_strides=(kk.stride(2), kk.stride(0)),
                     c_strides=(Sq * Skp, h * Sq * Skp), alpha=scale)
            ops.softmax(sc, pr, n0=nb, H=h, S=Sq, n=Sk, in_strides=(h * Sq * Skp, Sq * Skp, Skp),
                        out_strides=(h * Sq * Skp, Sq * Skp, Skp), rel_bias=rel_bias, rel_max=REL_MAX, causal=causal,
                        causal_off=Sk - Sq, window=window if causal else 0)
            ops.gemm(pr, vv, oo, M=Sq, N=dh, K=Sk, lda=Skp, ldb=vv.stride(1), ldc=oo.stride(1), zi=h, zo=nb,
                     b_zi_div=h // hk, a_strides=(Sq * Skp, h * Sq * Skp), b_strides=(vv.stride(2), vv.stride(0)),
                     c_strides=(dh, oo.stride(0)), b_mn=True)
        return out

    def encode_images(self, frames: torch.Tensor) -> torch.Tensor:
        g = self.g
        if frames.dim() != 5 or frames.shape[1] != 1 or g.image_channel != 1:
            raise NotImplementedError("single-channel volumes [F, 1, D, H, W] only")
        if list(frames.shape[2:]) != list(g.image_size):
            raise ValueError(f"frame size {list(frames.shape[2:])} != config.image_size {g.image_size}")
        Fr = frames.shape[0]
        Hd, P = g.vit_hidden, g.n_patches
        S = P + 1
        Sp = _pad8(S)
        vol = frames.to(device=self.dev, dtype=F32).contiguous().view(Fr, *g.image_size)
        x = torch.empty(Fr, Sp, Hd, device=self.dev, dtype=BF16)
        if self.fused_patch_embed and ops.patch_embed_supported(g.image_size, g.patch_size, Hd):
            ops.patch_embed(vol, g.patch_size, self.pe_w, self.pe_b, self.pos, x)
        else:
            rows = ops.patchify(vol, g.patch_size)
            ops.gemm(rows, self.pe_w, x, M=Fr * P, N=Hd, K=g.patch_dim, lda=g.patch_dim, ldb=g.patch_dim, ldc=Hd,
                     bias=self.pe_b, residual=self.pos, ldr=Hd, res_row_mod=P, row_remap=(P, Sp, 1))
            del rows
        ops.vit_frame_rows(x, self.cls, Fr, Sp, S)
        nh = g.vit_heads
        dh = Hd // nh
        x2 = x.view(Fr * Sp, Hd)
        y = torch.empty_like(x2)
        qkv = torch.empty(Fr * Sp, 3 * Hd, device=self.dev, dtype=BF16)
        ctx = torch.zeros(Fr, Sp, Hd, device=self.dev, dtype=BF16)
        hmid = torch.empty(Fr * Sp, g.vit_mlp, device=self.dev, dtype=BF16)
        qkv5 = qkv.view(Fr, Sp, 3, nh, dh)
        for w in self.vit:
            ops.layernorm(x2, w["ln1g"], w["ln1b"], 1e-5, out=y)
            ops.linear(y, w["wqkv"], w["bqkv"], out=qkv)
            self._attention(qkv5[:, :S, 0], qkv5[:, :S, 1], qkv5[:, :S, 2], ctx[:, :S], dh ** -0.5)
            ops.linear(ctx.view(Fr * Sp, Hd), w["wo"], w["bo"], residual=x2, out=x2)
            ops.layernorm(x2, w["ln2g"], w["ln2b"], 1e-5, out=y)
            ops.linear(y, w["w1"], w["b1"], act=ops.ACT_GELU, out=hmid)
            ops.linear(hmid, w["w2"], w["b2"], residual=x2, out=x2)
        ops.layernorm(x2, self.vit_ng, self.vit_nb, 1e-5, out=y)
        npf = g.tokens_per_frame
        pooled = torch.empty(Fr, npf, Hd, device=self.dev, dtype=BF16)
        ops.spp_pool(y, pooled, frames=Fr, grid=g.grid, ps=g.proj_pooling_size, E=Hd, in_frame_stride=Sp, in_off=1,
                     ldx=Hd, sequence=(g.proj_pooling_type == "sequence"))
        z = pooled.view(Fr * npf, Hd)
        n = len(self.proj)
        for i, (w, b) in enumerate(self.proj):
            act = ops.ACT_GELU if (g.proj_layer_type == "mlp" and i < n - 1) else ops.ACT_NONE
            z = ops.linear(z, w, b, act=act)
        return z.view(Fr, npf, g.hidden_size)

    def _u2t_self_attention(self, x2: torch.Tensor, nb: int, S: int, w: _SelfAttnW,
                            residual: Optional[torch.Tensor] = None) -> torch.Tensor:
        g = self.g
        E, H = g.hidden_size, g.u2t_num_heads
        dh = E // H
        qkv = ops.linear(x2, w.wqkv, w.bqkv)
        if g.attn_type == "rope":
            ops.rope(qkv, rows=nb * S, ld=3 * E, dh=dh, n_q=H, n_k=H, inv_freq=self.u2t_inv_freq, pos_div=1, pos_mod=S)
        q5 = qkv.view(nb, S, 3, H, dh)
        ctx = torch.empty(nb, S, E, device=self.dev, dtype=BF16)
        if w.seq_first:
            q5, ctx_v = q5.transpose(0, 1), ctx.transpose(0, 1)
            self._attention(q5[:, :, 0], q5[:, :, 1], q5[:, :, 2], ctx_v, 1.0 / math.sqrt(dh))
        else:
            self._attention(q5[:, :, 0], q5[:, :, 1], q5[:, :, 2], ctx, 1.0 / math.sqrt(dh), rel_bias=w.rel)
        return ops.linear(ctx.view(nb * S, E), w.wd, w.bd, residual=residual)

    def _u2t_temporal_attention(self, x2: torch.Tensor, B: int, C: int, N: int, w: _SelfAttnW) -> torch.Tensor:
        g = self.g
        E, H = g.hidden_size, g.u2t_num_heads
        dh = E // H
        qkv = ops.linear(x2, w.wqkv, w.bqkv)
        if w.seq_first:
            if B > 1:
                qkv = qkv.view(B, C, N, 3 * E).transpose(0, 1).contiguous()
            q5 = qkv.view(C, B * N, 3, H, dh)
            ctx = torch.empty(C, B * N, E, device=self.dev, dtype=BF16)
            self._attention(q5[:, :, 0], q5[:, :, 1], q5[:, :, 2], ctx, 1.0 / math.sqrt(dh))
            if B > 1:
                ctx = ctx.view(C, B, N, E).transpose(0, 1).contiguous()
            return ops.linear(ctx.view(B * C * N, E), w.wd, w.bd)
        if g.attn_type == "rope":
            ops.rope(qkv, rows=B * C * N, ld=3 * E, dh=dh, n_q=H, n_k=H, inv_freq=self.u2t_inv_freq, pos_div=N, pos_mod=C)
        ctx = torch.empty(B * C * N, E, device=self.dev, dtype=BF16)
        ops.temporal_attention(qkv, ctx, B=B, C_=C, N=N, H=H, dh=dh, scale=1.0 / math.sqrt(dh), rel_bias=w.rel,
                               rel_max=REL_MAX)
        return ops.linear(ctx, w.wd, w.bd)

    def _cross_attention(self, q_in: torch.Tensor, kv_in: torch.Tensor, B: int, Sq: int, Sk: int, w: _CrossAttnW,
                         residual: Optional[torch.Tensor]) -> torch.Tensor:
        g = self.g
        E, H = g.hidden_size, g.u2t_num_heads
        dh = E // H
        q = ops.linear(q_in, w.wq, w.bq).view(B, Sq, H, dh)
        ctx = torch.empty(B, Sq, E, device=self.dev, dtype=BF16)
        if w.wd is None:
            k = ops.linear(kv_in, w.wkv, w.bkv).view(B, Sk, H, dh)
            v = kv_in.view(B, Sk, H, dh)
            self._attention(q, k, v, ctx, 1.0 / math.sqrt(dh))
            return ctx.view(B * Sq, E)
        kv = ops.linear(kv_in, w.wkv, w.bkv).view(B, Sk, 2, H, dh)
        self._attention(q, kv[:, :, 0], kv[:, :, 1], ctx, 1.0 / math.sqrt(dh))
        return ops.linear(ctx.view(B * Sq, E), w.wd, w.bd, residual=residual)

    def _token_selection_diff(self, x2: torch.Tensor, B: int, T: int) -> torch.Tensor:
        g = self.g
        E, K = g.hidden_size, self.score_w.shape[0]
        Tp = _pad8(T)
        scT = torch.empty(K, B * T, device=self.dev, dtype=F32)
        ops.gemm(self.score_w, x2, scT, M=K, N=B * T, K=E, lda=E, ldb=E, ldc=B * T)
        pT = torch.empty(B, K, Tp, device=self.dev, dtype=BF16)
        ops.softmax(scT, pT, n0=B, H=1, S=K, n=T, in_strides=(T, 0, B * T), out_strides=(K * Tp, 0, Tp))
        sel = torch.empty(B, K, E, device=self.dev, dtype=BF16)
        ops.gemm(pT, x2, sel, M=K, N=E, K=T, lda=Tp, ldb=E, ldc=E, zo=B, a_strides=(0, K * Tp), b_strides=(0, T * E),
                 c_strides=(0, K * E), b_mn=True)
        return sel

    def _token_selection_hard(self, x2: torch.Tensor, B: int, T: int) -> torch.Tensor:
        g = self.g
        E, K = g.hidden_size, g.u2t_top_k
        if K > T:
            raise RuntimeError(f"selected index k out of range: top_k={K} > {T} tokens (torch.topk raises too)")
        sc = torch.empty(B * T, 1, device=self.dev, dtype=F32)
        ops.gemm(x2, self.score_w, sc, M=B * T, N=1, K=E, lda=E, ldb=E, ldc=1)
        idx = ops.topk_rows(sc.view(B, T), K, idx_offset_per_row=T)
        self.last_selection = idx
        return ops.embed_splice(idx, x2, None)

    def u2tokenizer(self, v_tokens: torch.Tensor, t_tokens: torch.Tensor) -> torch.Tensor:
# ... 653 lines not shown
```

### u2tokenizer_b200/ops.py

```python
from __future__ import annotations

import ctypes as C
from typing import Optional

import torch

from . import _lib
from ._lib import GemmDesc

BF16 = torch.bfloat16
F32 = torch.float32

ACT_NONE, ACT_GELU, ACT_SILU = 0, 1, 2
DT_BF16, DT_F32 = 0, 1


def _stream() -> int:
    return torch.cuda.current_stream().cuda_stream


def _ptr(t: Optional[torch.Tensor]) -> Optional[int]:
    return None if t is None else t.data_ptr()


def _need_cuda(*ts: torch.Tensor) -> None:
    for t in ts:
        if t is not None and not t.is_cuda:
            raise RuntimeError("u2tokenizer_b200 ops run on CUDA tensors only (no CPU fallback)")


def gemm(a: torch.Tensor, b: torch.Tensor, c: torch.Tensor, *, M: int, N: int, K: int,
         lda: int, ldb: int, ldc: int,
         zi: int = 1, zo: int = 1, b_zi_div: int = 1,
         a_strides=(0, 0), b_strides=(0, 0), c_strides=(0, 0),
         alpha: float = 1.0, bias: Optional[torch.Tensor] = None, act: int = ACT_NONE,
         residual: Optional[torch.Tensor] = None, ldr: int = 0, res_row_mod: int = 0,
         row_remap=(0, 0, 0), block_n: int = 0, a_mn: bool = False, b_mn: bool = False,
         epi_op: int = 0, rowvec: Optional[torch.Tensor] = None, rv_strides=(0, 0),
         mul: Optional[torch.Tensor] = None) -> torch.Tensor:
    _need_cuda(a, b, c, bias, residual)
    if a.dtype != BF16 or b.dtype != BF16:
        raise TypeError("gemm operands must be bf16")
    if c.dtype not in (BF16, F32):
        raise TypeError("gemm output must be bf16 or fp32")
    if bias is not None and bias.dtype != F32:
        raise TypeError("gemm bias must be fp32")
    if residual is not None and residual.dtype != BF16:
        raise TypeError("gemm residual must be bf16")
    d = GemmDesc()
    d.M, d.N, d.K = M, N, K
    d.zi, d.zo, d.b_zi_div = zi, zo, b_zi_div
    d.lda, d.a_stride_zi, d.a_stride_zo = lda, a_strides[0], a_strides[1]
    d.ldb, d.b_stride_zi, d.b_stride_zo = ldb, b_strides[0], b_strides[1]
    d.ldc, d.c_stride_zi, d.c_stride_zo = ldc, c_strides[0], c_strides[1]
    d.c_dtype = DT_BF16 if c.dtype == BF16 else DT_F32
    d.alpha = alpha
    d.bias = _ptr(bias)
    d.act = act
    d.residual = _ptr(residual)
    d.ldr = ldr
    d.res_row_mod = res_row_mod
    d.row_div, d.row_stride, d.row_off = row_remap
    d.block_n = block_n
    d.a_mn, d.b_mn = int(a_mn), int(b_mn)
    _need_cuda(rowvec, mul)
    d.epi_op = int(epi_op)
    d.rowvec = _ptr(rowvec)
    d.rv_stride_zi, d.rv_stride_zo = rv_strides
    d.mul = _ptr(mul)
    lib = _lib.load()
    if GEMM_TRACE is not None:
        e0, e1 = torch.cuda.Event(enable_timing=True), torch.cuda.Event(enable_timing=True)
        e0.record()
    _lib.check(lib.u2_gemm_bf16(a.data_ptr(), b.data_ptr(), c.data_ptr(), C.byref(d), _stream()),
               "u2_gemm_bf16")
    if GEMM_TRACE is not None:
        e1.record()
        GEMM_TRACE.append(((M, N, K, zi * zo, int(a_mn), int(b_mn), "f32" if c.dtype == F32 else "bf16", int(bias is not None),
                            int(act), int(residual is not None), int(epi_op)), e0, e1))
    return c


GEMM_TRACE = None


def linear(x: torch.Tensor, w: torch.Tensor, bias: Optional[torch.Tensor] = None, *,
           act: int = ACT_NONE, residual: Optional[torch.Tensor] = None,
           out: Optional[torch.Tensor] = None, out_dtype: torch.dtype = BF16,
           alpha: float = 1.0, block_n: int = 0) -> torch.Tensor:
    K = x.shape[-1]
    N = w.shape[0]
    if w.shape[1] != K:
        raise ValueError(f"linear: weight {tuple(w.shape)} does not match input K={K}")
    x2 = x.reshape(-1, K)
    if x2.stride(1) != 1:
        x2 = x2.contiguous()
    if w.stride(1) != 1:
        w = w.contiguous()
    M = x2.shape[0]
    if out is None:
        out = torch.empty(*x.shape[:-1], N, device=x.device, dtype=out_dtype)
    o2 = out.view(-1, N) if out.is_contiguous() else out
    r2 = None
    ldr = 0
    if residual is not None:
        r2 = residual.reshape(-1, N)
        if r2.stride(1) != 1:
            r2 = r2.contiguous()
        ldr = r2.stride(0)
    gemm(x2, w, o2, M=M, N=N, K=K, lda=x2.stride(0), ldb=w.stride(0), ldc=o2.stride(0),
         alpha=alpha, bias=bias, act=act, residual=r2, ldr=ldr, block_n=block_n)
    return out


def _rows2d(t: torch.Tensor) -> torch.Tensor:
    t2 = t.reshape(-1, t.shape[-1]) if t.dim() != 2 else t
    if t2.stride(1) != 1:
        raise ValueError("last dim must be contiguous")
    return t2


def layernorm(x, gamma, beta, eps=1e-5, residual=None, out=None, sum_out=None):
    _need_cuda(x, gamma, beta, residual)
    x2 = _rows2d(x)
    if out is None:
        out = torch.empty_like(x2)
    o2 = _rows2d(out)
    r2 = _rows2d(residual) if residual is not None else None
    s2 = _rows2d(sum_out) if sum_out is not None else None
    if s2 is not None and s2.stride(0) != o2.stride(0):
        raise ValueError("sum_out must share out's row stride")
    _lib.check(_lib.load().u2_layernorm_bf16(x2.data_ptr(), _ptr(r2), gamma.data_ptr(), _ptr(beta), o2.data_ptr(),
                                             _ptr(s2), x2.shape[0], x2.shape[1], x2.stride(0),
                                             r2.stride(0) if r2 is not None else 0, o2.stride(0), eps, _stream()),
               "u2_layernorm_bf16")
    return out.view(x.shape) if out.numel() == x.numel() and out.is_contiguous() else out


def rmsnorm(x, gamma, eps=1e-6, residual=None, out=None, sum_out=None):
    _need_cuda(x, gamma, residual)
    x2 = _rows2d(x)
    if out is None:
        out = torch.empty_like(x2)
    o2 = _rows2d(out)
    r2 = _rows2d(residual) if residual is not None else None
    s2 = _rows2d(sum_out) if sum_out is not None else None
    if s2 is not None and s2.stride(0) != o2.stride(0):
        raise ValueError("sum_out must share out's row stride")
    _lib.check(_lib.load().u2_rmsnorm_bf16(x2.data_ptr(), _ptr(r2), gamma.data_ptr(), o2.data_ptr(), _ptr(s2),
                                           x2.shape[0], x2.shape[1], x2.stride(0),
                                           r2.stride(0) if r2 is not None else 0, o2.stride(0), eps, _stream()),
               "u2_rmsnorm_bf16")
    return out.view(x.shape) if out.numel() == x.numel() and out.is_contiguous() else out


def softmax(scores: torch.Tensor, out: torch.Tensor, *, n0: int, H: int, S: int, n: int,
            in_strides, out_strides, scale: float = 1.0, rel_bias: Optional[torch.Tensor] = None,
            rel_max: int = 0, causal: bool = False, causal_off: int = 0, zero_pad_to: int = 0, window: int = 0):
    _need_cuda(scores, out, rel_bias)
    d = _lib.SoftmaxDesc()
    d.in_s0, d.in_s1, d.in_s2 = in_strides
    d.out_s0, d.out_s1, d.out_s2 = out_strides
    d.n0, d.H, d.S, d.n = n0, H, S, n
    d.scale = scale
    d.rel_bias = _ptr(rel_bias)
    d.rel_max = rel_max
    d.causal, d.causal_off = int(causal), causal_off
    d.zero_pad_to = zero_pad_to
    d.window = int(window or 0)
    _lib.check(_lib.load().u2_softmax_f32_bf16(scores.data_ptr(), out.data_ptr(), C.byref(d), _stream()),
               "u2_softmax_f32_bf16")
    return out


def silu_mul(gate_up: torch.Tensor, out: Optional[torch.Tensor] = None, interleaved: bool = False) -> torch.Tensor:
    _need_cuda(gate_up)
    g2 = _rows2d(gate_up)
    I = g2.shape[1] // 2
    if out is None:
        out = torch.empty(g2.shape[0], I, device=g2.device, dtype=BF16)
    _lib.check(_lib.load().u2_silu_mul_bf16(g2.data_ptr(), out.data_ptr(), g2.shape[0], I, g2.stride(0),
                                            out.stride(0), int(interleaved), _stream()), "u2_silu_mul_bf16")
    return out


def patchify(vol: torch.Tensor, patch_size, out: Optional[torch.Tensor] = None) -> torch.Tensor:
    _need_cuda(vol)
    if vol.dtype != F32 or not vol.is_contiguous():
        raise TypeError("patchify expects a contiguous fp32 volume")
    F_, d0, d1, d2 = vol.shape
    p0, p1, p2 = patch_size
    npatch = (d0 // p0) * (d1 // p1) * (d2 // p2)
    if out is None:
        out = torch.empty(F_ * npatch, p0 * p1 * p2, device=vol.device, dtype=BF16)
    _lib.check(_lib.load().u2_patchify_f32_bf16(vol.data_ptr(), out.data_ptr(), F_, d0, d1, d2, p0, p1, p2,
                                                _stream()), "u2_patchify_f32_bf16")
    return out


def patch_embed_supported(image_size, patch_size, hidden: int) -> bool:
    d0, d1, d2 = image_size
    p0, p1, p2 = patch_size
    if d0 % p0 or d1 % p1 or d2 % p2:
        return False
    return p2 == 16 and d2 // p2 == 16 and p1 % 4 == 0 and (d1 // p1) % 8 == 0 and d2 <= 256 and hidden % 32 == 0


def patch_embed(vol: torch.Tensor, patch_size, w: torch.Tensor, bias: torch.Tensor, pos: torch.Tensor,
                out: torch.Tensor) -> torch.Tensor:
    _need_cuda(vol, w, bias, pos, out)
    if vol.dtype != F32 or not vol.is_contiguous() or w.dtype != BF16 or bias.dtype != F32 or pos.dtype != BF16:
        raise TypeError("patch_embed: fp32 contiguous volume, bf16 weight / position table, fp32 bias")
    F_, d0, d1, d2 = vol.shape
    p0, p1, p2 = patch_size
    N = w.shape[0]
    if out.shape[0] != F_ or out.shape[2] != N or not out.is_contiguous() or not w.is_contiguous() or not pos.is_contiguous():
        raise ValueError("patch_embed: out must be contiguous [frames, rows, N]")
    _lib.check(_lib.load().u2_patch_embed_f32_bf16(vol.data_ptr(), w.data_ptr(), bias.data_ptr(), pos.data_ptr(), out.data_ptr(),
                                                   F_, d0, d1, d2, p0, p1, p2, N, out.shape[1], _stream()),
               "u2_patch_embed_f32_bf16")
    return out


def set_rows(dst: torch.Tensor, vec: torch.Tensor, n_rows: int, row_stride: int, row_off: int):
    _need_cuda(dst, vec)
    E = vec.numel()
    _lib.check(_lib.load().u2_set_rows_bf16(dst.data_ptr(), vec.data_ptr(), n_rows, row_stride, row_off, E,
                                            _stream()), "u2_set_rows_bf16")
    return dst


def vit_frame_rows(dst: torch.Tensor, cls: torch.Tensor, frames: int, Sp: int, S: int):
    _need_cuda(dst, cls)
    _lib.check(_lib.load().u2_vit_frame_rows_bf16(dst.data_ptr(), cls.data_ptr(), frames, Sp, S, cls.numel(), _stream()),
               "u2_vit_frame_rows_bf16")
    return dst


def transpose_heads(x: torch.Tensor, out: torch.Tensor, *, B: int, S: int, H: int, Dh: int,
                    in_strides, out_strides, ld_out: int):
    _need_cuda(x, out)
    _lib.check(_lib.load().u2_transpose_heads_bf16(x.data_ptr(), out.data_ptr(), B, S, H, Dh, in_strides[0],
                                                   in_strides[1], in_strides[2], out_strides[0], out_strides[1],
                                                   ld_out, _stream()), "u2_transpose_heads_bf16")
    return out


def spp_pool(x: torch.Tensor, out: torch.Tensor, *, frames: int, grid, ps: int, E: int,
             in_frame_stride: int, in_off: int, ldx: int, sequence: bool = False):
    _need_cuda(x, out)
    _lib.check(_lib.load().u2_spp_pool_bf16(x.data_ptr(), out.data_ptr(), frames, grid[0], grid[1], grid[2], ps, E,
                                            in_frame_stride, in_off, ldx, int(sequence), _stream()),
               "u2_spp_pool_bf16")
    return out


def multiscale_pool(x: torch.Tensor, gate_w: Optional[torch.Tensor], gate_bias: float, dynamic: bool) -> torch.Tensor:
    _need_cuda(x, gate_w)
    B, K, E = x.shape
    x = x.contiguous()
    n_out = K + (K // 2 if K >= 2 else 0) + (K // 4 if K >= 4 else 0)
    out = torch.empty(B, n_out, E, device=x.device, dtype=BF16)
    ws = torch.empty(int(_lib.load().u2_multiscale_pool_ws_elems(B, K)), device=x.device, dtype=F32)
    _lib.check(_lib.load().u2_multiscale_pool_bf16(x.data_ptr(), out.data_ptr(), _ptr(gate_w), gate_bias,
                                                   ws.data_ptr(), B, K, E, int(dynamic), _stream()),
               "u2_multiscale_pool_bf16")
    return out


def embed_splice(ids: torch.Tensor, table: torch.Tensor, vis: Optional[torch.Tensor],
                 out: Optional[torch.Tensor] = None) -> torch.Tensor:
    _need_cuda(ids, table, vis)
    if ids.dtype != torch.int64:
        ids = ids.long()
    ids = ids.contiguous()
    B, L = ids.shape
    E = table.shape[1]
    n_vis = 0 if vis is None else vis.shape[1]
    if vis is not None:
        vis = vis.contiguous()
    if out is None:
        out = torch.empty(B, L, E, device=table.device, dtype=BF16)
    _lib.check(_lib.load().u2_embed_splice_bf16(ids.data_ptr(), table.data_ptr(), _ptr(vis), out.data_ptr(), B, L, E,
                                                n_vis, table.shape[0], _stream()), "u2_embed_splice_bf16")
    return out


def temporal_attention(qkv: torch.Tensor, out: torch.Tensor, *, B: int, C_: int, N: int, H: int, dh: int,
                       scale: float, rel_bias: Optional[torch.Tensor], rel_max: int = 512):
    _need_cuda(qkv, out, rel_bias)
    _lib.check(_lib.load().u2_temporal_attention_bf16(qkv.data_ptr(), out.data_ptr(), B, C_, N, H, dh,
                                                      qkv.stride(-2), out.stride(-2), scale, _ptr(rel_bias),
                                                      rel_max, _stream()), "u2_temporal_attention_bf16")
    return out


def rope(x: torch.Tensor, *, rows: int, ld: int, dh: int, n_q: int, n_k: int, n_v: int = 0,
         inv_freq: torch.Tensor, q_norm_w=None, k_norm_w=None, eps: float = 1e-6,
         pos0: int = 0, pos_div: int = 1, pos_mod: int = 1, pos0_dev=None,
         k_cache=None, v_cache=None, Tmax: int = 0, rows_per_batch: int = 1, pos0_per_batch: bool = False):
    _need_cuda(x, inv_freq, q_norm_w, k_norm_w, k_cache, v_cache, pos0_dev)
    d = _lib.RopeDesc()
    d.rows, d.ld, d.dh = rows, ld, dh
    d.n_q_heads, d.n_k_heads, d.n_v_heads = n_q, n_k, n_v
    d.q_norm_w, d.k_norm_w, d.eps = _ptr(q_norm_w), _ptr(k_norm_w), eps
    d.inv_freq = inv_freq.data_ptr()
    d.pos0, d.pos_div, d.pos_mod = pos0, pos_div, pos_mod
    d.pos0_dev = _ptr(pos0_dev)
    d.k_cache, d.v_cache = _ptr(k_cache), _ptr(v_cache)
    d.Tmax, d.rows_per_batch = Tmax, rows_per_batch
    d.pos0_per_batch = 1 if pos0_per_batch else 0
    _lib.check(_lib.load().u2_rope_bf16(x.data_ptr(), C.byref(d), _stream()), "u2_rope_bf16")
    return x


def decode_attention(q: torch.Tensor, k_cache: torch.Tensor, v_cache: torch.Tensor, out: torch.Tensor, *,
                     B: int, Hq: int, Hkv: int, dh: int, Tmax: int, T: int = 0, T_dev=None, ldq: int, ldo: int,
                     scale: float, T_per_seq: bool = False, kv_src: Optional[torch.Tensor] = None, window: int = 0):
    _need_cuda(q, k_cache, v_cache, out, T_dev, kv_src)
    _check_kv_src(kv_src, B, Tmax)
    if window:
        _lib.check(_lib.load().u2_decode_attention_window_bf16(
            q.data_ptr(), k_cache.data_ptr(), v_cache.data_ptr(), out.data_ptr(), B, Hq, Hkv, dh, Tmax, T, _ptr(T_dev),
            ldq, ldo, scale, 1 if T_per_seq else 0, _ptr(kv_src), kv_src.stride(0) if kv_src is not None else 0,
            int(window), _stream()), "u2_decode_attention_window_bf16")
        return out
    _lib.check(_lib.load().u2_decode_attention_bf16(q.data_ptr(), k_cache.data_ptr(), v_cache.data_ptr(),
                                                    out.data_ptr(), B, Hq, Hkv, dh, Tmax, T, _ptr(T_dev), ldq, ldo,
                                                    scale, 1 if T_per_seq else 0, _ptr(kv_src),
                                                    kv_src.stride(0) if kv_src is not None else 0, _stream()),
               "u2_decode_attention_bf16")
    return out


def _check_kv_src(kv_src: Optional[torch.Tensor], B: int, Tmax: int) -> None:
    if kv_src is not None and (kv_src.dtype != torch.int32 or kv_src.dim() != 2 or kv_src.shape[0] != B
                               or kv_src.shape[1] < Tmax or kv_src.stride(1) != 1):
        raise ValueError(f"kv_src must be int32 [{B}, >= {Tmax}] with unit column stride")


def gemv(x: torch.Tensor, w: torch.Tensor, out: torch.Tensor, *, residual=None, norm_gamma=None,
         norm_eps: float = 1e-6, silu_pair: bool = False):
    _need_cuda(x, w, out, residual, norm_gamma)
    d = _lib.GemvDesc()
    d.B, d.N, d.K = x.shape[0], w.shape[0], w.shape[1]
    d.ldx, d.ldw, d.ldy = x.stride(0), w.stride(0), out.stride(0)
    d.ldr = residual.stride(0) if residual is not None else 0
    d.y_dtype = DT_BF16 if out.dtype == BF16 else DT_F32
    d.residual = _ptr(residual)
    d.norm_gamma = _ptr(norm_gamma)
    d.norm_eps = norm_eps
    d.silu_pair = int(silu_pair)
    _lib.check(_lib.load().u2_gemv_bf16(x.data_ptr(), w.data_ptr(), out.data_ptr(), C.byref(d), _stream()),
               "u2_gemv_bf16")
    return out


_argmax_scratch = {}


def argmax(logits: torch.Tensor, out: Optional[torch.Tensor] = None) -> torch.Tensor:
    _need_cuda(logits)
    B, V = logits.shape
    if out is None:
        out = torch.empty(B, device=logits.device, dtype=torch.int64)
    sc = _argmax_scratch.get(logits.device)
    if sc is None:
        sc = _argmax_scratch[logits.device] = torch.zeros(1024, device=logits.device, dtype=torch.int64)
    _lib.check(_lib.load().u2_argmax_f32(logits.data_ptr(), out.data_ptr(), sc.data_ptr(), B, V, logits.stride(0),
                                         _stream()), "u2_argmax_f32")
    return out


def _dlinear_desc(x, w, out, *, ws, counters, ssq_in=None, eps=1e-6, residual=None, silu_pair=False, gamma_next=None,
                  xg=None, ssq_out=None, ssq_zero=None, pdl=True, dbg=None, sched=0, dep_flags=None, dep_shift=1,
                  out_flags=None):
    _need_cuda(x, w, out, ws, counters, ssq_in, residual, gamma_next, xg, ssq_out, ssq_zero)
    d = _lib.DlinearDesc()
    d.B, d.N, d.K = x.shape[0], w.shape[0], w.shape[1]
    if counters.numel() < (d.N + 63) // 64 + (ssq_out is not None):
        raise ValueError("dlinear counters too small: ceil(N / 64) int32, + 1 with ssq_out")
    d.ws_elems = ws.numel()
    d.ldx, d.ldw, d.ldy = x.stride(0), w.stride(0), out.stride(0)
    d.ldr = residual.stride(0) if residual is not None else 0
    d.ldxg = xg.stride(0) if xg is not None else 0
    d.y_dtype = DT_BF16 if out.dtype == BF16 else DT_F32
    d.ws, d.counters = ws.data_ptr(), counters.data_ptr()
    d.ssq_in = _ptr(ssq_in)
    d.eps = eps
    d.residual = _ptr(residual)
    d.silu_pair = int(silu_pair)
    d.gamma_next = _ptr(gamma_next)
    d.xg = _ptr(xg)
    d.ssq_out = _ptr(ssq_out)
    d.ssq_zero = _ptr(ssq_zero)
    d.pdl = int(pdl)
    d.dbg = _ptr(dbg)
    _need_cuda(dep_flags, out_flags)
    d.dep_flags, d.dep_shift, d.out_flags = _ptr(dep_flags), dep_shift, _ptr(out_flags)
    d.sched = int(sched)
    return d


def dlinear_ws_elems(N: int, K: int) -> int:
    return int(_lib.load().u2_dlinear_ws_elems(N, K))


def dlinear_new_ws(n_elems: int, device="cuda", lead=()) -> torch.Tensor:
    return torch.full((*lead, max(int(n_elems), 4)), -1, device=device, dtype=torch.int32).view(F32)


def dlinear(x: torch.Tensor, w: torch.Tensor, out: torch.Tensor, **kw):
    d = _dlinear_desc(x, w, out, **kw)
    _lib.check(_lib.load().u2_dlinear_bf16(x.data_ptr(), w.data_ptr(), out.data_ptr(), C.byref(d), _stream()),
               "u2_dlinear_bf16")
    return out


def dlinear_multi(ops_list, *, gridbar: torch.Tensor, step_dev: torch.Tensor, pdl: bool = True,
                  lookahead_units: int = 0, next_weights=(), pre_stages: int = 0):
    n = len(ops_list)
    descs = (_lib.DlinearDesc * n)()
    xs, ws_, ys = (C.c_void_p * n)(), (C.c_void_p * n)(), (C.c_void_p * n)()
    for i, (x, w, out, kw) in enumerate(ops_list):
        descs[i] = _dlinear_desc(x, w, out, **kw)
        xs[i], ws_[i], ys[i] = x.data_ptr(), w.data_ptr(), out.data_ptr()
    _need_cuda(gridbar, step_dev)
    nx = _lib.DlinearNext()
    nx.lookahead_units = lookahead_units
    nx.pre_stages = pre_stages
    nx.n = len(next_weights)
    for j, (wn, units) in enumerate(next_weights):
        _need_cuda(wn)
        nx.w[j], nx.N[j], nx.K[j], nx.ldw[j], nx.units[j] = wn.data_ptr(), wn.shape[0], wn.shape[1], wn.stride(0), units
    _lib.check(_lib.load().u2_dlinear_multi_bf16(xs, ws_, ys, descs, n, gridbar.data_ptr(), step_dev.data_ptr(),
                                                 int(pdl), C.byref(nx), _stream()), "u2_dlinear_multi_bf16")


def decode_embed(ids: torch.Tensor, table: torch.Tensor, gamma: torch.Tensor, x: torch.Tensor, xg: torch.Tensor,
                 ssq: torch.Tensor, ssq_zero: Optional[torch.Tensor], step_counter: Optional[torch.Tensor] = None):
    _need_cuda(ids, table, gamma, x, xg, ssq, ssq_zero, step_counter)
    _lib.check(_lib.load().u2_decode_embed_bf16(ids.data_ptr(), table.data_ptr(), gamma.data_ptr(), x.data_ptr(),
                                                xg.data_ptr(), ssq.data_ptr(), _ptr(ssq_zero), _ptr(step_counter),
                                                ids.numel(),
                                                table.shape[1], table.shape[0], _stream()), "u2_decode_embed_bf16")
    return x


def decode_attention_fused(qkv: torch.Tensor, k_cache: torch.Tensor, v_cache: torch.Tensor, out: torch.Tensor, *,
                           B: int, Hq: int, Hkv: int, dh: int, Tmax: int, inv_freq: torch.Tensor, scale: float,
                           pos: int = 0, pos_dev=None, q_norm_w=None, k_norm_w=None, eps: float = 1e-6, kv_splits: int = 1,
                           pdl: bool = False, pos_per_seq: bool = False, kv_src: Optional[torch.Tensor] = None,
                           window: int = 0):
    _need_cuda(qkv, k_cache, v_cache, out, inv_freq, pos_dev, q_norm_w, k_norm_w, kv_src)
    _check_kv_src(kv_src, B, Tmax)
    d = _lib.FusedDecodeDesc()
    d.B, d.Hq, d.Hkv, d.dh, d.Tmax, d.pos = B, Hq, Hkv, dh, Tmax, pos
    d.pos_dev = _ptr(pos_dev)
    d.ldq, d.ldo = qkv.stride(0), out.stride(0)
    d.q_norm_w, d.k_norm_w, d.eps = _ptr(q_norm_w), _ptr(k_norm_w), eps
    d.inv_freq = inv_freq.data_ptr()
    d.scale = scale
    d.kv_splits = int(kv_splits)
    d.pdl = 1 if pdl else 0
    d.pos_per_seq = 1 if pos_per_seq else 0
    d.kv_src = _ptr(kv_src)
    d.ld_kv_src = kv_src.stride(0) if kv_src is not None else 0
    d.window = int(window or 0)
    _lib.check(_lib.load().u2_decode_attention_fused_bf16(qkv.data_ptr(), k_cache.data_ptr(), v_cache.data_ptr(),
                                                          out.data_ptr(), C.byref(d), _stream()),
               "u2_decode_attention_fused_bf16")
    return out


def topk_rows(scores: torch.Tensor, k: int, idx_offset_per_row: int = 0) -> torch.Tensor:
    _need_cuda(scores)
    if scores.dtype != F32 or scores.stride(1) != 1:
        raise TypeError("topk_rows expects fp32 rows")
    rows, T = scores.shape
    out = torch.empty(rows, k, device=scores.device, dtype=torch.int64)
    _lib.check(_lib.load().u2_topk_rows_f32(scores.data_ptr(), out.data_ptr(), rows, T, k, scores.stride(0),
                                            idx_offset_per_row, _stream()), "u2_topk_rows_f32")
    return out


def flash_attention_d64(q: torch.Tensor, k: torch.Tensor, v: torch.Tensor, out: torch.Tensor, scale: float,
                        lse: Optional[torch.Tensor] = None):
    _need_cuda(q, k, v, out)
    B, Sq, H, dh = q.shape
    Sk = k.shape[1]
    if dh != 64 or q.stride(3) != 1 or k.stride(3) != 1 or v.stride(3) != 1 or out.stride(2) != 1 or v.shape != k.shape:
        raise ValueError("flash_attention_d64: head_dim must be 64 with a contiguous last dim, v shaped like k")
    d = _lib.FaDesc()
    d.B, d.H, d.Sq, d.Sk, d.dh, d.scale = B, H, Sq, Sk, dh, scale
    d.q_sb, d.q_ss, d.q_sh = q.stride(0), q.stride(1), q.stride(2)
    d.k_sb, d.k_ss, d.k_sh = k.stride(0), k.stride(1), k.stride(2)
    d.v_sb, d.v_ss, d.v_sh = v.stride(0), v.stride(1), v.stride(2)
    d.out_sb, d.out_ss = out.stride(0), out.stride(1)
    _need_cuda(lse)
    if lse is not None and (lse.dtype != F32 or not lse.is_contiguous() or lse.numel() != B * H * Sq):
        raise ValueError("flash_attention_d64: lse must be contiguous fp32 [B, H, Sq]")
    d.lse = _ptr(lse)
    _lib.check(_lib.load().u2_flash_attention_d64_bf16(q.data_ptr(), k.data_ptr(), v.data_ptr(), out.data_ptr(),
                                                       C.byref(d), _stream()), "u2_flash_attention_d64_bf16")
    return out


def sample(logits: torch.Tensor, out: Optional[torch.Tensor] = None, *, temperature: float = 1.0, top_k: int = 50,
           top_p: float = 1.0, seed: int = 0, step: int = 0, step_dev=None) -> torch.Tensor:
    _need_cuda(logits, step_dev)
    B, V = logits.shape
    if out is None:
        out = torch.empty(B, device=logits.device, dtype=torch.int64)
    _lib.check(_lib.load().u2_sample_f32(logits.data_ptr(), out.data_ptr(), B, V, logits.stride(0), temperature,
                                         int(top_k), float(top_p), int(seed) & ((1 << 64) - 1), _ptr(step_dev),
                                         int(step), _stream()), "u2_sample_f32")
    return out


def sample_params(device, temperature: float, top_k: int, top_p: float, seed: int,
                  out: Optional[torch.Tensor] = None) -> torch.Tensor:
    import struct
    if not temperature > 0:
        raise ValueError("sample: temperature must be > 0")
    if not 0 < top_p <= 1:
        raise ValueError("sample: top_p must be in (0, 1]")
    raw = struct.pack("<fifiQ", float(temperature), int(top_k), float(top_p), 0, int(seed) & ((1 << 64) - 1))
    host = torch.frombuffer(bytearray(raw), dtype=torch.uint8)
    if out is None:
        return host.to(device)
    out.copy_(host)
    return out


def sample_dev(logits: torch.Tensor, params: torch.Tensor, out: Optional[torch.Tensor] = None, *, step: int = 0,
               step_dev=None) -> torch.Tensor:
    _need_cuda(logits, params, step_dev)
    B, V = logits.shape
    if params.dtype != torch.uint8 or params.numel() != 24:
        raise ValueError("sample_dev: params must be the 24-byte block of sample_params()")
    if out is None:
        out = torch.empty(B, device=logits.device, dtype=torch.int64)
    _lib.check(_lib.load().u2_sample_dev_f32(logits.data_ptr(), out.data_ptr(), B, V, logits.stride(0), params.data_ptr(),
                                             _ptr(step_dev), int(step), _stream()), "u2_sample_dev_f32")
    return out


def logits_proc_params(device, vocab_size: int, *, repetition_penalty: float = 1.0, no_repeat_ngram_size: int = 0,
                       min_new_tokens: int = 0, eos_token_ids=(), bad_words_ids=(),
                       out: Optional[torch.Tensor] = None) -> torch.Tensor:
    import numpy as np
    p = float(repetition_penalty)
    if not p > 0:
        raise ValueError(f"repetition_penalty must be > 0, got {repetition_penalty}")
    n, k = int(no_repeat_ngram_size), int(min_new_tokens)
    if n < 0 or k < 0:
        raise ValueError("no_repeat_ngram_size and min_new_tokens must be >= 0")
    eos = [int(e) for e in eos_token_ids]
    words = [[int(x) for x in w] for w in bad_words_ids]
    if len(eos) > _lib.LP_MAX_EOS:
        raise ValueError(f"at most {_lib.LP_MAX_EOS} EOS ids, got {len(eos)}")
    if len(words) > _lib.LP_MAX_BAD_WORDS or sum(map(len, words)) > _lib.LP_MAX_BAD_TOKENS:
        raise ValueError(f"bad_words_ids holds at most {_lib.LP_MAX_BAD_WORDS} words of "
                         f"{_lib.LP_MAX_BAD_TOKENS} tokens in all")
    if any(len(w) == 0 for w in words):
        raise ValueError("bad_words_ids: every word needs at least one token")
    bad = [v for v in eos + [x for w in words for x in w] if not 0 <= v < vocab_size]
    if bad:
        raise ValueError(f"token ids {bad} outside the vocabulary [0, {vocab_size})")
    blk = _lib.LogitsProcParams()
    blk.penalty = p
    blk.inv_penalty = float(np.float32(1.0) / np.float32(p))
    blk.ngram, blk.min_new, blk.n_eos, blk.n_bad = n, k, len(eos), len(words)
    for i, e in enumerate(eos):
        blk.eos[i] = e
    off = 0
    for i, w in enumerate(words):
        blk.bad_off[i] = off
        for x in w:
            blk.bad_tok[off] = x
            off += 1
    blk.bad_off[len(words)] = off
    host = torch.frombuffer(bytearray(bytes(blk)), dtype=torch.uint8)
    if out is None:
        return host.to(device)
    out.copy_(host)
    return out


def logits_process(logits: torch.Tensor, params: torch.Tensor, ids: torch.Tensor, hist: torch.Tensor, *,
                   step: int = 0, step_dev=None) -> torch.Tensor:
    _need_cuda(logits, params, ids, hist, step_dev)
    B, V = logits.shape
    if logits.dtype != F32 or logits.stride(1) != 1:
        raise TypeError("logits_process: logits must be fp32 with unit column stride")
    if params.dtype != torch.uint8 or params.numel() != C.sizeof(_lib.LogitsProcParams):
        raise ValueError("logits_process: params must be the block of logits_proc_params()")
    if ids.dtype != torch.int64 or ids.numel() != B or not ids.is_contiguous():
        raise ValueError("logits_process: ids must be contiguous int64 [B]")
    if hist.dtype != torch.int32 or hist.dim() != 2 or hist.shape[0] != B or hist.stride(1) != 1:
        raise ValueError("logits_process: hist must be int32 [B, cap] with unit column stride")
    if step_dev is None and not 0 <= step <= hist.shape[1]:
        raise ValueError(f"logits_process: step {step} outside the history capacity {hist.shape[1]}")
    _lib.check(_lib.load().u2_logits_process_f32(logits.data_ptr(), B, V, logits.stride(0), ids.data_ptr(),
                                                 hist.data_ptr(), hist.stride(0), hist.shape[1], params.data_ptr(),
                                                 _ptr(step_dev), int(step), _stream()), "u2_logits_process_f32")
    return logits


def log_softmax(x: torch.Tensor, out: Optional[torch.Tensor] = None) -> torch.Tensor:
    _need_cuda(x, out)
    if x.dtype != F32 or x.dim() != 2 or x.stride(1) != 1:
        raise TypeError("log_softmax expects fp32 rows with unit column stride")
    if out is None:
        out = torch.empty_like(x)
    if out.dtype != F32 or out.shape != x.shape or out.stride(1) != 1:
        raise ValueError("log_softmax: out must be fp32 shaped like x")
    _lib.check(_lib.load().u2_log_softmax_f32(x.data_ptr(), out.data_ptr(), x.shape[0], x.shape[1], x.stride(0),
                                              out.stride(0), _stream()), "u2_log_softmax_f32")
    return out


EARLY_STOPPING = {False: 0, True: 1, "never": 2}


def beam_params(device, *, num_beams: int, length_penalty: float = 1.0, early_stopping=False, max_new_tokens: int,
                eos_token_ids=(), out: Optional[torch.Tensor] = None) -> torch.Tensor:
    K, eos = int(num_beams), [int(e) for e in eos_token_ids]
    if not 2 <= K <= _lib.BEAM_MAX_BEAMS:
        raise ValueError(f"num_beams must be in 2..{_lib.BEAM_MAX_BEAMS}, got {num_beams}")
    if len(eos) > _lib.BEAM_MAX_EOS:
        raise ValueError(f"beam search supports at most {_lib.BEAM_MAX_EOS} EOS ids, got {len(eos)}")
    if not (early_stopping is True or early_stopping is False or early_stopping == "never"):
        raise ValueError(f"early_stopping must be True, False or 'never', got {early_stopping!r}")
    if int(max_new_tokens) < 1:
        raise ValueError("max_new_tokens must be >= 1")
    blk = _lib.BeamParams()
    blk.length_penalty = float(length_penalty)
    blk.num_beams, blk.beams_to_keep = K, max(2, 1 + len(eos)) * K
    blk.early_stopping, blk.max_new_tokens, blk.n_eos = EARLY_STOPPING[early_stopping], int(max_new_tokens), len(eos)
    for i, e in enumerate(eos):
        blk.eos[i] = e
    host = torch.frombuffer(bytearray(bytes(blk)), dtype=torch.uint8)
    if out is None:
        return host.to(device)
    out.copy_(host)
    return out


def beam_topk(logprobs: torch.Tensor, running: torch.Tensor, flags: torch.Tensor, params: torch.Tensor,
              cand_val: torch.Tensor, cand_tok: torch.Tensor):
    _need_cuda(logprobs, running, flags, params, cand_val, cand_tok)
    R, V = logprobs.shape
    if logprobs.dtype != F32 or logprobs.stride(1) != 1:
        raise TypeError("beam_topk: fp32 log-probs with unit column stride")
    if cand_val.shape != (R, _lib.BEAM_MAX_KEEP) or cand_tok.shape != (R, _lib.BEAM_MAX_KEEP):
        raise ValueError(f"beam_topk: candidates must be [{R}, {_lib.BEAM_MAX_KEEP}]")
    _lib.check(_lib.load().u2_beam_topk_f32(logprobs.data_ptr(), logprobs.stride(0), R, V, running.data_ptr(),
                                            flags.data_ptr(), params.data_ptr(), cand_val.data_ptr(),
                                            cand_tok.data_ptr(), _stream()), "u2_beam_topk_f32")


def beam_step(params: torch.Tensor, st: dict, ids: torch.Tensor, kv_src: torch.Tensor, pos_dev: torch.Tensor, *,
              V: int, hist: Optional[torch.Tensor] = None, step: int = 0, step_dev=None):
    d = _lib.BeamStepDesc()
    d.params = params.data_ptr()
    d.prompts, d.V = st["flags"].shape[0], int(V)
    for k in ("cand_val", "cand_tok", "running", "fin_score", "fin_info", "flags"):
        _need_cuda(st[k])
        setattr(d, k, st[k].data_ptr())
    _need_cuda(ids, kv_src, pos_dev, hist, step_dev)
    if ids.dtype != torch.int64 or kv_src.dtype != torch.int32 or not kv_src.is_contiguous():
        raise ValueError("beam_step: ids int64, kv_src contiguous int32")
    d.ids = ids.data_ptr()
    d.rec, d.ld_rec, d.rec_rows = st["rec"].data_ptr(), st["rec"].stride(0), st["rec"].shape[0]
    d.kv_src, d.ld_kv_src = kv_src.data_ptr(), kv_src.stride(0)
    d.pos_dev = pos_dev.data_ptr()
    if hist is not None:
        d.hist, d.ld_hist, d.hist_cap = hist.data_ptr(), hist.stride(0), hist.shape[1]
    d.step_dev = _ptr(step_dev)
    _lib.check(_lib.load().u2_beam_step(C.byref(d), int(step), _stream()), "u2_beam_step")


def lmhead_logprob(hidden: torch.Tensor, weight: torch.Tensor, labels: torch.Tensor, *, want_lse: bool = False,
                   want_logit_sum: bool = False, nll_acc: Optional[torch.Tensor] = None, ws: Optional[torch.Tensor] = None):
    _need_cuda(hidden, weight, labels, nll_acc, ws)
    R, E = hidden.shape
    V = weight.shape[0]
    if hidden.dtype != torch.bfloat16 or weight.dtype != torch.bfloat16 or labels.dtype != torch.int64:
        raise TypeError("lmhead_logprob: hidden / weight must be bf16, labels int64")
    if weight.shape[1] != E or labels.shape != (R,) or hidden.stride(1) != 1 or weight.stride(1) != 1 or not labels.is_contiguous():
        raise ValueError("lmhead_logprob: shape / stride mismatch")
    lib = _lib.load()
    need = int(lib.u2_logprob_ws_bytes(R, V))
    if ws is None:
        ws = torch.empty(need, device=hidden.device, dtype=torch.uint8)
    elif ws.numel() * ws.element_size() < need:
        raise ValueError(f"lmhead_logprob: workspace of {need} bytes required")
    logp = torch.empty(R, device=hidden.device, dtype=torch.float32)
    lse = torch.empty(R, device=hidden.device, dtype=torch.float32) if want_lse else None
    lsum = torch.empty(R, device=hidden.device, dtype=torch.float32) if want_logit_sum else None
    d = _lib.LogprobDesc()
    d.R, d.V, d.E, d.ldh, d.ldw = R, V, E, hidden.stride(0), weight.stride(0)
    d.labels, d.ws, d.ws_bytes = labels.data_ptr(), ws.data_ptr(), ws.numel() * ws.element_size()
    d.lse, d.logit_sum, d.nll_acc = _ptr(lse), _ptr(lsum), _ptr(nll_acc)
    _lib.check(lib.u2_lmhead_logprob_bf16(hidden.data_ptr(), weight.data_ptr(), logp.data_ptr(), C.byref(d), _stream()),
# ... 35 lines not shown
```

Before: 2.133.

## Add cluster split-K dlinear schedule with DSMEM partial-sum reduction

Adds a new dlinear schedule in which each thread block cluster owns a contiguous range of 64-row tiles and splits K across its CTAs. Non-finalizer CTAs send their partial accumulators to the finalizer over distributed shared memory using st.async with mbarrier completion, replacing global-workspace stream-K reduction for that schedule. The default schedule stays stream-K 128, and the default stage count for the 128-row config drops from 10 to 8. The new path adds cluster barriers and receive buffers, which increase shared memory use.

```diff
diff --git a/include/u2b200.h b/include/u2b200.h
--- a/include/u2b200.h
+++ b/include/u2b200.h
@@ -148,6 +148,7 @@
 
 #define U2_DLIN_STREAMK128 0
 #define U2_DLIN_TILES64 1
+#define U2_DLIN_CLUSTER64 2
 typedef struct u2_dlinear_desc {
   int32_t B, N, K;
   int64_t ldx, ldw, ldy, ldr, ldxg;
@@ -171,6 +172,7 @@
   int32_t sched;
 } u2_dlinear_desc;
 U2_API int u2_dlinear_bf16(const void* x, const void* w, void* y, const u2_dlinear_desc* desc, void* stream);
+U2_API int32_t u2_dlinear_clusters(int32_t* cluster_size);
 U2_API int64_t u2_dlinear_ws_elems(int32_t N, int32_t K);
 typedef struct u2_dlinear_next {
   int32_t pre_stages;
diff --git a/u2tokenizer_b200/_lib.py b/u2tokenizer_b200/_lib.py
--- a/u2tokenizer_b200/_lib.py
+++ b/u2tokenizer_b200/_lib.py
@@ -265,6 +265,7 @@
     "u2_beam_topk_f32": (C.c_int, [_P, _L, _I, _I, _P, _P, _P, _P, _P, _P]),
     "u2_beam_step": (C.c_int, [C.POINTER(BeamStepDesc), _I, _P]),
     "u2_dlinear_ws_elems": (C.c_int64, [_I, _I]),
+    "u2_dlinear_clusters": (C.c_int32, [_P]),
     "u2_dlinear_multi_bf16": (C.c_int, [_P, _P, _P, _P, _I, _P, _P, _I, _P, _P]),
     "u2_preprocess_ws_bytes": (C.c_int64, [_I, _I, _I]),
     "u2_preprocess_volume_f32": (C.c_int, [_P, _P, _P, C.POINTER(PreprocessDesc), _P]),
diff --git a/u2tokenizer_b200/csrc/dlinear_wgmma.cu b/u2tokenizer_b200/csrc/dlinear_wgmma.cu
--- a/u2tokenizer_b200/csrc/dlinear_wgmma.cu
+++ b/u2tokenizer_b200/csrc/dlinear_wgmma.cu
@@ -16,16 +16,19 @@
 constexpr int kDlMmaWarp0 = 8;
 constexpr int kDlAccLd = 20;
 
-template <int kM>
+constexpr int kDlClusterMax = 4;
+
+template <int kM, bool kCl = false>
 struct DlCfg {
   static constexpr int kABytes = kM * kDlK * 2;
   static constexpr int kStageBytes = kABytes + kDlBBytes;
 #ifndef U2_DL_STAGES128
-#define U2_DL_STAGES128 10
+#define U2_DL_STAGES128 8
 #endif
   static constexpr int kStages = (kM == 128) ? U2_DL_STAGES128 : 18;
   static constexpr int kAccBytes = 2 * kM * kDlAccLd * 4;
-  static constexpr int kSmem = kStages * kStageBytes + kAccBytes + 1024 + 512;
+  static constexpr int kRecvBytes = kCl ? 2 * (kDlClusterMax - 1) * kM * kDlN * 4 : 0;
+  static constexpr int kSmem = kStages * kStageBytes + kAccBytes + kRecvBytes + 1024 + 512;
 };
 
 struct DlinArgs {
@@ -111,10 +114,11 @@
 
 struct UnitIter {
   int tile, kb, kblocks, tile_step;
+  int kb0;
   int left;
   __device__ __forceinline__ void next() {
     if (++kb == kblocks) {
-      kb = 0;
+      kb = kb0;
       tile += tile_step;
     }
     --left;
@@ -125,10 +129,34 @@
   }
 };
 
+struct ClusterPart {
+  int t0, t1, k0, k1;
+};
+
+__device__ __forceinline__ ClusterPart cluster_part(int num_tiles, int kblocks) {
+  const int c = (int)cluster_id_x(), nc = (int)cluster_count_x();
+  const int r = (int)cluster_ctarank(), C = (int)cluster_nctarank();
+  ClusterPart cp;
+  cp.t0 = (int)((long long)num_tiles * c / nc);
+  cp.t1 = (int)((long long)num_tiles * (c + 1) / nc);
+  cp.k0 = kblocks * r / C;
+  cp.k1 = kblocks * (r + 1) / C;
+  return cp;
+}
+
+template <bool kCl>
 __device__ __forceinline__ UnitIter make_iter(int num_tiles, int kblocks, bool tiles) {
   UnitIter it;
   it.kblocks = kblocks;
-  if (tiles) {
+  it.kb0 = 0;
+  if (kCl) {
+    const ClusterPart cp = cluster_part(num_tiles, kblocks);
+    it.tile = cp.t0;
+    it.kb = it.kb0 = cp.k0;
+    it.kblocks = cp.k1;
+    it.tile_step = 1;
+    it.left = (cp.t1 - cp.t0) * (cp.k1 - cp.k0);
+  } else if (tiles) {
     const int mine = (num_tiles > (int)blockIdx.x) ? (num_tiles - (int)blockIdx.x + (int)gridDim.x - 1) / (int)gridDim.x : 0;
     it.tile = blockIdx.x;
     it.kb = 0;
@@ -172,10 +200,132 @@
   asm volatile("fence.proxy.async;" ::: "memory");
 }
 
+__device__ __forceinline__ void cluster_bar_wait(uint64_t* bar, uint32_t parity, const char* what) {
+  unsigned int spins = 0;
+  while (!mbar_try_wait_cluster(bar, parity)) {
+    if (++spins == (1u << 26)) {
+      printf("u2 dlinear: %s wait timed out (CTA %d, cluster rank %u)\n", what, (int)blockIdx.x, cluster_ctarank());
+      __trap();
+    }
+  }
+}
+
+__device__ __forceinline__ void load_tile_operands(const DlinArgs& p, int row, bool row_ok, unsigned short (&res_raw)[16],
+                                                   float (&rs)[16], float& gam) {
+#pragma unroll
+  for (int b = 0; b < 16; ++b) {
+    res_raw[b] = 0;
+    rs[b] = 1.f;
+    if (b < p.B) {
+      if (p.residual && !p.silu_pair && row_ok)
+        res_raw[b] = __ldcg(reinterpret_cast<const unsigned short*>(p.residual) + (long long)b * p.ldr + row);
+      if (p.ssq_in) rs[b] = __ldcg(p.ssq_in + b);
+    }
+  }
+  if (p.gamma_next && row_ok) gam = __ldg(p.gamma_next + row);
+}
+
 template <int kM>
+__device__ __forceinline__ void finish_tile(const DlinArgs& p, int tile, int trow, bool tvalid, float (&f)[16],
+                                            const unsigned short (&res_raw)[16], const float (&rs)[16], float gam,
+                                            unsigned int target) {
+  const int et = threadIdx.x - 128;
+  const int lane = threadIdx.x % 32;
+  const int q = (threadIdx.x / 32) - 4;
+  const int row = tile * kM + trow;
+  const bool row_ok = tvalid && row < p.N;
+  if (p.ssq_zero && tile == 0 && et < 16) p.ssq_zero[et] = 0.f;
+  float sq[16];
+#pragma unroll
+  for (int b = 0; b < 16; ++b) {
+    sq[b] = 0.f;
+    if (b < p.B) {
+      float val = f[b];
+      if (p.ssq_in) val *= rsqrtf(rs[b] * p.inv_norm_dim + p.eps);
+      if (p.silu_pair) {
+        const float me = __bfloat162float(__float2bfloat16(val));
+        const float other = __shfl_down_sync(0xffffffffu, me, 1);
+        if (row_ok && (trow & 1) == 0) {
+          const float o = __fdividef(me, 1.f + __expf(-me)) * other;
+          reinterpret_cast<__nv_bfloat16*>(p.y)[(long long)b * p.ldy + (row >> 1)] = __float2bfloat16(o);
+        }
+      } else if (row_ok) {
+        val += __bfloat162float(__ushort_as_bfloat16(res_raw[b]));
+        if (p.y_dtype == U2_DT_BF16) {
+          const __nv_bfloat16 o = __float2bfloat16(val);
+          reinterpret_cast<__nv_bfloat16*>(p.y)[(long long)b * p.ldy + row] = o;
+          val = __bfloat162float(o);
+        } else {
+          reinterpret_cast<float*>(p.y)[(long long)b * p.ldy + row] = val;
+        }
+        if (p.gamma_next) p.xg[(long long)b * p.ldxg + row] = __float2bfloat16(val * gam);
+        sq[b] = val * val;
+      }
+    }
+  }
+  if (p.ssq_out) {
+    __shared__ float s_sq[4][16];
+    __shared__ int s_last;
+#pragma unroll
+    for (int b = 0; b < 16; ++b) {
+      float s = sq[b];
+#pragma unroll
+      for (int o = 16; o > 0; o >>= 1) s += __shfl_xor_sync(0xffffffffu, s, o);
+      if (lane == 0) s_sq[q][b] = s;
+    }
+    asm volatile("bar.sync 1, 128;" ::: "memory");
+    if (et < 16) {
+      __stcg(p.ssq_part + (long long)tile * 16 + et, ((s_sq[0][et] + s_sq[1][et]) + s_sq[2][et]) + s_sq[3][et]);
+      __threadfence();
+    }
+    asm volatile("bar.sync 1, 128;" ::: "memory");
+    if (et == 0) s_last = (atomicAdd(p.ssq_ticket, 1) == p.num_tiles - 1);
+    asm volatile("bar.sync 1, 128;" ::: "memory");
+    if (s_last) {
+      __shared__ float s_grp[8][16];
+      __threadfence();
+      const int col = et & 15, grp = et >> 4;
+      float t = 0.f;
+      for (int i0 = grp; i0 < p.num_tiles; i0 += 32) {
+        float v[4];
+#pragma unroll
+        for (int u = 0; u < 4; ++u) {
+          const int i = i0 + 8 * u;
+          v[u] = (i < p.num_tiles) ? __ldcg(p.ssq_part + (long long)i * 16 + col) : 0.f;
+        }
+#pragma unroll
+        for (int u = 0; u < 4; ++u) {
+          const int i = i0 + 8 * u;
+          if (i < p.num_tiles) {
+            t += v[u];
+            __stcg(p.ssq_part + (long long)i * 16 + col, __uint_as_float(0xffffffffu));
+          }
+        }
+      }
+      s_grp[grp][col] = t;
+      asm volatile("bar.sync 1, 128;" ::: "memory");
+      if (et < p.B) {
+        float tot = 0.f;
+#pragma unroll
+        for (int g = 0; g < 8; ++g) tot += s_grp[g][et];
+        p.ssq_out[et] += tot;
+      }
+      if (et == 0) *p.ssq_ticket = 0;
+    }
+  }
+  if (p.out_flags) {
+    asm volatile("bar.sync 1, 128;" ::: "memory");
+    if (et == 0) {
+      const int stepv = (int)(target / gridDim.x);
+      asm volatile("st.release.gpu.global.s32 [%0], %1;" ::"l"(p.out_flags + tile), "r"(stepv) : "memory");
+    }
+  }
+}
+
+template <int kM, bool kCl>
 __global__ void __launch_bounds__(kDlThreads, 1)
 dlinear_wgmma_kernel(const __grid_constant__ DlinMulti mp) {
-  using Cfg = DlCfg<kM>;
+  using Cfg = DlCfg<kM, kCl>;
   constexpr int kStages = Cfg::kStages;
   constexpr int kABytes = Cfg::kABytes;
   constexpr int kStageBytes = Cfg::kStageBytes;
@@ -185,11 +335,14 @@
   uint8_t* smem_a = smem;
   uint8_t* smem_b = smem + kStages * kABytes;
   float* smem_acc = reinterpret_cast<float*>(smem + kStages * kStageBytes);
-  uint64_t* bars = reinterpret_cast<uint64_t*>(smem + kStages * kStageBytes + Cfg::kAccBytes);
+  float* smem_recv = reinterpret_cast<float*>(smem + kStages * kStageBytes + Cfg::kAccBytes);
+  uint64_t* bars = reinterpret_cast<uint64_t*>(smem + kStages * kStageBytes + Cfg::kAccBytes + Cfg::kRecvBytes);
   uint64_t* full_bar = bars;
   uint64_t* empty_bar = bars + kStages;
   uint64_t* acc_full_bar = bars + 2 * kStages;
   uint64_t* acc_empty_bar = bars + 2 * kStages + 2;
+  uint64_t* recv_full_bar = bars + 2 * kStages + 4;
+  uint64_t* recv_free_bar = bars + 2 * kStages + 6;
   __shared__ unsigned char s_ready[1024];
   if (threadIdx.x < 256) reinterpret_cast<unsigned int*>(s_ready)[threadIdx.x] = 0u;
 
@@ -212,9 +365,16 @@
       mbar_init(&acc_full_bar[s], 4);
       mbar_init(&acc_empty_bar[s], 4);
     }
+    if (kCl) {
+      for (int s = 0; s < 2; ++s) mbar_init(&recv_full_bar[s], 1);
+      for (int s = 0; s < 2 * kDlClusterMax; ++s) mbar_init(&recv_free_bar[s], 1);
+    }
     fence_barrier_init();
   }
-  __syncthreads();
+  if (kCl)
+    cluster_sync_all();
+  else
+    __syncthreads();
   asm volatile("griddepcontrol.launch_dependents;" ::: "memory");
 
   if (warp_idx == 0) {
@@ -226,7 +386,7 @@
       int step = 0;
       for (int oi = 0; oi < n_ops; ++oi) {
         const DlinArgs& p = mp.op[oi];
-        UnitIter it = make_iter(p.num_tiles, p.kblocks, kTiles);
+        UnitIter it = make_iter<kCl>(p.num_tiles, p.kblocks, kTiles);
         const int pre_cap = (oi == 0 || mp.pre_stages <= 0 || mp.pre_stages > kStages) ? kStages : mp.pre_stages;
         const int npre = it.left < pre_cap ? it.left : pre_cap;
         int st = stage;
@@ -282,7 +442,7 @@
         }
       }
       for (int jn = 0; jn < mp.n_next; ++jn) {
-        UnitIter la = make_iter(mp.next_tiles[jn], mp.next_kblocks[jn], kTiles);
+        UnitIter la = make_iter<kCl>(mp.next_tiles[jn], mp.next_kblocks[jn], kTiles);
         for (int j = 0; j < mp.next_units[jn] && la.left > 0; ++j) {
           tma_prefetch_l2_4d(&mp.tnext[jn], la.kb * kDlK, la.tile * kM, 0, 0);
           la.next();
@@ -296,7 +456,7 @@
     int acc = 0;
     uint32_t acc_phase = 0;
     for (int oi = 0; oi < n_ops; ++oi) {
-      UnitIter it = make_iter(mp.op[oi].num_tiles, mp.op[oi].kblocks, kTiles);
+      UnitIter it = make_iter<kCl>(mp.op[oi].num_tiles, mp.op[oi].kblocks, kTiles);
       bool first_unit = true;
       while (it.left > 0) {
         const int seg = it.seg_len();
@@ -353,211 +513,197 @@
     const unsigned int target = (unsigned int)(*reinterpret_cast<const volatile int*>(mp.step_dev)) * gridDim.x;
     int acc = 0;
     uint32_t acc_phase = 0;
+    const int crank = kCl ? (int)cluster_ctarank() : 0;
+    const int csize = kCl ? (int)cluster_nctarank() : 1;
+    int sent[kDlClusterMax] = {0, 0, 0, 0};
+    int fin = 0;
     for (int oi = 0; oi < n_ops; ++oi) {
       const DlinArgs& p = mp.op[oi];
-      UnitIter it = make_iter(p.num_tiles, p.kblocks, kTiles);
+      UnitIter it = make_iter<kCl>(p.num_tiles, p.kblocks, kTiles);
       bool prev_done = (oi == 0);
       if (oi > 0 && !p.dep_flags) {
         if (et == 0) grid_barrier_wait(mp.gridbar + (oi - 1), target);
         asm volatile("bar.sync 1, 128;" ::: "memory");
         prev_done = true;
       }
-      while (it.left > 0) {
-        const int tile = it.tile;
-        const int seg_kb = it.seg_len();
-        it.left -= seg_kb;
-        it.kb += seg_kb;
-        if (it.kb == it.kblocks) {
-          it.kb = 0;
-          it.tile += it.tile_step;
-        }
-
-        const int row = tile * kM + trow;
-        const bool whole = (seg_kb == p.kblocks);
-        int gf = (int)blockIdx.x, n_contrib = 0;
-        if (!whole) {
-          const long long units = (long long)p.num_tiles * p.kblocks;
-          const long long G = units < (long long)gridDim.x ? units : (long long)gridDim.x;
-          const long long u0 = (long long)tile * p.kblocks;
-          gf = (int)(((u0 + 1) * G + units - 1) / units) - 1;
-          n_contrib = (int)(((u0 + p.kblocks) * G + units - 1) / units) - 1 - gf;
-        }
-        const bool finalizer = (gf == (int)blockIdx.x);
-        const int nvec = (p.B + 3) >> 2;
-        const bool row_ok = tvalid && row < p.N;
-        unsigned short res_raw[16];
-        float rs[16];
-        float gam = 0.f;
-        if (finalizer) {
-          if (!prev_done) {
-            if (et == 0) grid_barrier_wait(mp.gridbar + (oi - 1), target);
+      if constexpr (kCl) {
+        const ClusterPart cp = cluster_part(p.num_tiles, p.kblocks);
+        const bool has = cp.k1 > cp.k0;
+        for (int tile = cp.t0; tile < cp.t1; ++tile) {
+          const int fr = tile % csize;
+          const bool finalizer = (fr == crank);
+          const int row = tile * kM + trow;
+          const bool row_ok = tvalid && row < p.N;
+          unsigned short res_raw[16];
+          float rs[16];
+          float gam = 0.f;
+          if (finalizer) load_tile_operands(p, row, row_ok, res_raw, rs, gam);
+          float f[16];
+          if (has) {
+            mbar_wait(&acc_full_bar[acc], acc_phase);
+            if (et == 0 && tile + 1 == cp.t1) U2_STAMP(oi, 4);
+            const uint32_t src = smem_u32(smem_acc + acc * (kM * kDlAccLd) + trow * kDlAccLd);
+#pragma unroll
+            for (int c = 0; c < 4; ++c) {
+              const float4 x = lds128_f32(src + 16 * c);
+              f[4 * c] = x.x; f[4 * c + 1] = x.y; f[4 * c + 2] = x.z; f[4 * c + 3] = x.w;
+            }
+            __syncwarp();
+            if ((threadIdx.x & 31) == 0) mbar_arrive(&acc_empty_bar[acc]);
+            if (++acc == 2) {
+              acc = 0;
+              acc_phase ^= 1;
+            }
+          } else {
+#pragma unroll
+            for (int b = 0; b < 16; ++b) f[b] = 0.f;
+          }
+          if (!finalizer) {
+            const int bf = sent[fr] & 1;
+            cluster_bar_wait(&recv_free_bar[fr * 2 + bf], ((sent[fr] >> 1) & 1) ^ 1, "receive buffer");
+            ++sent[fr];
+            if (tvalid) {
+              const int slot = crank < fr ? crank : crank - 1;
+              const uint32_t dst =
+                  mapa_shared(smem_u32(smem_recv + ((bf * (kDlClusterMax - 1) + slot) * kM + trow) * kDlN), (uint32_t)fr);
+              const uint32_t bar = mapa_shared(smem_u32(&recv_full_bar[bf]), (uint32_t)fr);
+#pragma unroll
+              for (int c = 0; c < 4; ++c) st_async_f4(dst + 16 * c, f[4 * c], f[4 * c + 1], f[4 * c + 2], f[4 * c + 3], bar);
+            }
+          } else {
+            const int bf = fin & 1;
+            if (et == 0) U2_STAMP(oi, 6);
+            if (et == 0) mbar_arrive_expect_tx(&recv_full_bar[bf], (uint32_t)((csize - 1) * kM * kDlN * 4));
+            cluster_bar_wait(&recv_full_bar[bf], (fin >> 1) & 1, "partial tile");
+            ++fin;
+            float t[16];
+#pragma unroll 1
+            for (int s = 0; s < csize; ++s) {
+              float g[16];
+              if (s == crank) {
+#pragma unroll
+                for (int b = 0; b < 16; ++b) g[b] = f[b];
+              } else {
+                const int slot = s < crank ? s : s - 1;
+                const uint32_t src = smem_u32(smem_recv + ((bf * (kDlClusterMax - 1) + slot) * kM + trow) * kDlN);
+#pragma unroll
+                for (int c = 0; c < 4; ++c) {
+                  const float4 x = lds128_f32(src + 16 * c);
+                  g[4 * c] = x.x; g[4 * c + 1] = x.y; g[4 * c + 2] = x.z; g[4 * c + 3] = x.w;
+                }
+              }
+#pragma unroll
+              for (int b = 0; b < 16; ++b) t[b] = (s == 0) ? g[b] : t[b] + g[b];
+            }
             asm volatile("bar.sync 1, 128;" ::: "memory");
-            prev_done = true;
-          }
-#pragma unroll
-          for (int b = 0; b < 16; ++b) {
-            res_raw[b] = 0;
-            rs[b] = 1.f;
-            if (b < p.B) {
-              if (p.residual && !p.silu_pair && row_ok)
-                res_raw[b] = __ldcg(reinterpret_cast<const unsigned short*>(p.residual) + (long long)b * p.ldr + row);
-              if (p.ssq_in) rs[b] = __ldcg(p.ssq_in + b);
+            if (et < csize && et != crank) mbar_arrive_remote(mapa_shared(smem_u32(&recv_free_bar[crank * 2 + bf]), (uint32_t)et));
+            if (et == 0) U2_STAMP(oi, 7);
+            finish_tile<kM>(p, tile, trow, tvalid, t, res_raw, rs, gam, target);
+          }
+        }
+      } else {
+        while (it.left > 0) {
+          const int tile = it.tile;
+          const int seg_kb = it.seg_len();
+          it.left -= seg_kb;
+          it.kb += seg_kb;
+          if (it.kb == it.kblocks) {
+            it.kb = 0;
+            it.tile += it.tile_step;
+          }
+
+          const int row = tile * kM + trow;
+          const bool whole = (seg_kb == p.kblocks);
+          int gf = (int)blockIdx.x, n_contrib = 0;
+          if (!whole) {
+            const long long units = (long long)p.num_tiles * p.kblocks;
+            const long long G = units < (long long)gridDim.x ? units : (long long)gridDim.x;
+            const long long u0 = (long long)tile * p.kblocks;
+            gf = (int)(((u0 + 1) * G + units - 1) / units) - 1;
+            n_contrib = (int)(((u0 + p.kblocks) * G + units - 1) / units) - 1 - gf;
+          }
+          const bool finalizer = (gf == (int)blockIdx.x);
+          const int nvec = (p.B + 3) >> 2;
+          const bool row_ok = tvalid && row < p.N;
+          unsigned short res_raw[16];
+          float rs[16];
+          float gam = 0.f;
+          if (finalizer) {
+            if (!prev_done) {
+              if (et == 0) grid_barrier_wait(mp.gridbar + (oi - 1), target);
+              asm volatile("bar.sync 1, 128;" ::: "memory");
+              prev_done = true;
             }
-          }
-          if (p.gamma_next && row_ok) gam = __ldg(p.gamma_next + row);
-        }
-
-        mbar_wait(&acc_full_bar[acc], acc_phase);
-        if (et == 0 && it.left == 0) U2_STAMP(oi, 4);
-        uint32_t v[16];
-        {
-          const uint32_t src = smem_u32(smem_acc + acc * (kM * kDlAccLd) + trow * kDlAccLd);
-#pragma unroll
-          for (int c = 0; c < 4; ++c) {
-            const uint4 x = lds128(src + 16 * c);
-            v[4 * c] = x.x; v[4 * c + 1] = x.y; v[4 * c + 2] = x.z; v[4 * c + 3] = x.w;
-          }
-        }
-        __syncwarp();
-        if ((threadIdx.x & 31) == 0) mbar_arrive(&acc_empty_bar[acc]);
-        if (++acc == 2) {
-          acc = 0;
-          acc_phase ^= 1;
-        }
-
-        float f[16];
-#pragma unroll
-        for (int b = 0; b < 16; ++b) f[b] = __uint_as_float(v[b]);
-        if (!finalizer) {
-          const int slot = (int)blockIdx.x - gf - 1;
-          float4* dst = reinterpret_cast<float4*>(p.ws + (((long long)tile * p.max_slots + slot) * kM + trow) * kDlN);
-          if (tvalid) {
-#pragma unroll
-            for (int c = 0; c < 4; ++c)
-              if (c < nvec) __stcg(dst + c, make_float4(f[4 * c], f[4 * c + 1], f[4 * c + 2], f[4 * c + 3]));
-          }
-        } else {
-          if (et == 0) U2_STAMP(oi, 6);
-          if (n_contrib > 0 && tvalid) {
-            const long long slot_stride = (long long)kM * kDlN / 4;
-            float4* src0 = reinterpret_cast<float4*>(p.ws + (((long long)tile * p.max_slots) * kM + trow) * kDlN);
-            const float4 sent = make_float4(__uint_as_float(0xffffffffu), __uint_as_float(0xffffffffu),
-                                            __uint_as_float(0xffffffffu), __uint_as_float(0xffffffffu));
-#pragma unroll
+            load_tile_operands(p, row, row_ok, res_raw, rs, gam);
+          }
+
+          mbar_wait(&acc_full_bar[acc], acc_phase);
+          if (et == 0 && it.left == 0) U2_STAMP(oi, 4);
+          uint32_t v[16];
+          {
+            const uint32_t src = smem_u32(smem_acc + acc * (kM * kDlAccLd) + trow * kDlAccLd);
+  #pragma unroll
             for (int c = 0; c < 4; ++c) {
-              if (c >= nvec) break;
-              constexpr int kMaxSlots = 8;
-              for (int s0 = 0; s0 < n_contrib; s0 += kMaxSlots) {
-                float4 t[kMaxSlots];
-                bool ok;
-                unsigned int spins = 0;
-                do {
-                  ok = true;
-#pragma unroll
-                  for (int sl = 0; sl < kMaxSlots; ++sl)
-                    if (s0 + sl < n_contrib) t[sl] = ld_relaxed_f4(src0 + (s0 + sl) * slot_stride + c);
-#pragma unroll
+              const uint4 x = lds128(src + 16 * c);
+              v[4 * c] = x.x; v[4 * c + 1] = x.y; v[4 * c + 2] = x.z; v[4 * c + 3] = x.w;
+            }
+          }
+          __syncwarp();
+          if ((threadIdx.x & 31) == 0) mbar_arrive(&acc_empty_bar[acc]);
+          if (++acc == 2) {
+            acc = 0;
+            acc_phase ^= 1;
+          }
+
+          float f[16];
+  #pragma unroll
+          for (int b = 0; b < 16; ++b) f[b] = __uint_as_float(v[b]);
+          if (!finalizer) {
+            const int slot = (int)blockIdx.x - gf - 1;
+            float4* dst = reinterpret_cast<float4*>(p.ws + (((long long)tile * p.max_slots + slot) * kM + trow) * kDlN);
+            if (tvalid) {
+  #pragma unroll
+              for (int c = 0; c < 4; ++c)
+                if (c < nvec) __stcg(dst + c, make_float4(f[4 * c], f[4 * c + 1], f[4 * c + 2], f[4 * c + 3]));
+            }
+          } else {
+            if (et == 0) U2_STAMP(oi, 6);
+            if (n_contrib > 0 && tvalid) {
+              const long long slot_stride = (long long)kM * kDlN / 4;
+              float4* src0 = reinterpret_cast<float4*>(p.ws + (((long long)tile * p.max_slots) * kM + trow) * kDlN);
+              const float4 sent = make_float4(__uint_as_float(0xffffffffu), __uint_as_float(0xffffffffu),
+                                              __uint_as_float(0xffffffffu), __uint_as_float(0xffffffffu));
+  #pragma unroll
+              for (int c = 0; c < 4; ++c) {
+                if (c >= nvec) break;
+                constexpr int kMaxSlots = 8;
+                for (int s0 = 0; s0 < n_contrib; s0 += kMaxSlots) {
+                  float4 t[kMaxSlots];
+                  bool ok;
+                  unsigned int spins = 0;
+                  do {
+                    ok = true;
+  #pragma unroll
+                    for (int sl = 0; sl < kMaxSlots; ++sl)
+                      if (s0 + sl < n_contrib) t[sl] = ld_relaxed_f4(src0 + (s0 + sl) * slot_stride + c);
+  #pragma unroll
+                    for (int sl = 0; sl < kMaxSlots; ++sl)
+                      if (s0 + sl < n_contrib) {
+                        ok = ok && (__float_as_uint(t[sl].x) != 0xffffffffu) && (__float_as_uint(t[sl].y) != 0xffffffffu) &&
+                             (__float_as_uint(t[sl].z) != 0xffffffffu) && (__float_as_uint(t[sl].w) != 0xffffffffu);
+                      }
+                  } while (!ok && ++spins < (1u << 22));
+  #pragma unroll
                   for (int sl = 0; sl < kMaxSlots; ++sl)
                     if (s0 + sl < n_contrib) {
-                      ok = ok && (__float_as_uint(t[sl].x) != 0xffffffffu) && (__float_as_uint(t[sl].y) != 0xffffffffu) &&
-                           (__float_as_uint(t[sl].z) != 0xffffffffu) && (__float_as_uint(t[sl].w) != 0xffffffffu);
+                      f[4 * c] += t[sl].x; f[4 * c + 1] += t[sl].y; f[4 * c + 2] += t[sl].z; f[4 * c + 3] += t[sl].w;
+                      __stcg(src0 + (s0 + sl) * slot_stride + c, sent);
                     }
-                } while (!ok && ++spins < (1u << 22));
-#pragma unroll
-                for (int sl = 0; sl < kMaxSlots; ++sl)
-                  if (s0 + sl < n_contrib) {
-                    f[4 * c] += t[sl].x; f[4 * c + 1] += t[sl].y; f[4 * c + 2] += t[sl].z; f[4 * c + 3] += t[sl].w;
-                    __stcg(src0 + (s0 + sl) * slot_stride + c, sent);
-                  }
+                }
               }
             }
-          }
-          if (et == 0) U2_STAMP(oi, 7);
-          if (p.ssq_zero && tile == 0 && et < 16) p.ssq_zero[et] = 0.f;
-          float sq[16];
-#pragma unroll
-          for (int b = 0; b < 16; ++b) {
-            sq[b] = 0.f;
-            if (b < p.B) {
-              float val = f[b];
-              if (p.ssq_in) val *= rsqrtf(rs[b] * p.inv_norm_dim + p.eps);
-              if (p.silu_pair) {
-                const float me = __bfloat162float(__float2bfloat16(val));
-                const float other = __shfl_down_sync(0xffffffffu, me, 1);
-                if (row_ok && (trow & 1) == 0) {
-                  const float o = __fdividef(me, 1.f + __expf(-me)) * other;
-                  reinterpret_cast<__nv_bfloat16*>(p.y)[(long long)b * p.ldy + (row >> 1)] = __float2bfloat16(o);
-                }
-              } else if (row_ok) {
-                val += __bfloat162float(__ushort_as_bfloat16(res_raw[b]));
-                if (p.y_dtype == U2_DT_BF16) {
-                  const __nv_bfloat16 o = __float2bfloat16(val);
-                  reinterpret_cast<__nv_bfloat16*>(p.y)[(long long)b * p.ldy + row] = o;
-                  val = __bfloat162float(o);
-                } else {
-                  reinterpret_cast<float*>(p.y)[(long long)b * p.ldy + row] = val;
-                }
-                if (p.gamma_next) p.xg[(long long)b * p.ldxg + row] = __float2bfloat16(val * gam);
-                sq[b] = val * val;
-              }
-            }
-          }
-          if (p.ssq_out) {
-            __shared__ float s_sq[4][16];
-            __shared__ int s_last;
-#pragma unroll
-            for (int b = 0; b < 16; ++b) {
-              float s = sq[b];
-#pragma unroll
-              for (int o = 16; o > 0; o >>= 1) s += __shfl_xor_sync(0xffffffffu, s, o);
-              if (lane == 0) s_sq[q][b] = s;
-            }
-            asm volatile("bar.sync 1, 128;" ::: "memory");
-            if (et < 16) {
-              __stcg(p.ssq_part + (long long)tile * 16 + et, ((s_sq[0][et] + s_sq[1][et]) + s_sq[2][et]) + s_sq[3][et]);
-              __threadfence();
-            }
-            asm volatile("bar.sync 1, 128;" ::: "memory");
-            if (et == 0) s_last = (atomicAdd(p.ssq_ticket, 1) == p.num_tiles - 1);
-            asm volatile("bar.sync 1, 128;" ::: "memory");
-            if (s_last) {
-              __shared__ float s_grp[8][16];
-              __threadfence();
-              const int col = et & 15, grp = et >> 4;
-              float t = 0.f;
-              for (int i0 = grp; i0 < p.num_tiles; i0 += 32) {
-                float v[4];
-#pragma unroll
-                for (int u = 0; u < 4; ++u) {
-                  const int i = i0 + 8 * u;
-                  v[u] = (i < p.num_tiles) ? __ldcg(p.ssq_part + (long long)i * 16 + col) : 0.f;
-                }
-#pragma unroll
-                for (int u = 0; u < 4; ++u) {
-                  const int i = i0 + 8 * u;
-                  if (i < p.num_tiles) {
-                    t += v[u];
-                    __stcg(p.ssq_part + (long long)i * 16 + col, __uint_as_float(0xffffffffu));
-                  }
-                }
-              }
-              s_grp[grp][col] = t;
-              asm volatile("bar.sync 1, 128;" ::: "memory");
-              if (et < p.B) {
-                float tot = 0.f;
-#pragma unroll
-                for (int g = 0; g < 8; ++g) tot += s_grp[g][et];
-                p.ssq_out[et] += tot;
-              }
-              if (et == 0) *p.ssq_ticket = 0;
-            }
-          }
-          if (p.out_flags) {
-            asm volatile("bar.sync 1, 128;" ::: "memory");
-            if (et == 0) {
-              const int stepv = (int)(target / gridDim.x);
-              asm volatile("st.release.gpu.global.s32 [%0], %1;" ::"l"(p.out_flags + tile), "r"(stepv) : "memory");
-            }
+            if (et == 0) U2_STAMP(oi, 7);
+            finish_tile<kM>(p, tile, trow, tvalid, f, res_raw, rs, gam, target);
           }
         }
       }
@@ -568,6 +714,7 @@
       }
     }
   }
+  if (kCl) cluster_sync_all();
 }
 
 __global__ void __launch_bounds__(256)
@@ -614,6 +761,8 @@
   if ((d->ldx & 7) || (d->ldw & 7)) return set_error(U2_ERR_ARG, "dlinear: ldx/ldw must be multiples of 8");
   if (d->silu_pair && (d->N & 1)) return set_error(U2_ERR_ARG, "dlinear: silu_pair needs an even N");
   if (d->gamma_next && !d->xg) return set_error(U2_ERR_ARG, "dlinear: gamma_next needs xg");
+  if (d->sched == U2_DLIN_CLUSTER64 && d->dep_flags)
+    return set_error(U2_ERR_ARG, "dlinear: per-tile dependency flags need the stream-K schedule");
   p->B = d->B; p->N = d->N; p->K = d->K;
   p->num_tiles = (d->N + kM - 1) / kM;
   p->kblocks = d->K / kDlK;
@@ -662,46 +811,121 @@
   return make_tmap_bf16_4d(tx, x, d->K, d->B, 1, 1, d->ldx, 0, 0, kDlK, kDlN);
 }
 
-template <int kM>
-static int launch_multi_t(DlinMulti& mp, int pdl, cudaStream_t stream) {
+template <int kM, bool kCl>
+static int configure_kernel() {
   static bool configured = false;
   if (!configured) {
-    cudaError_t e = cudaFuncSetAttribute(dlinear_wgmma_kernel<kM>, cudaFuncAttributeMaxDynamicSharedMemorySize, DlCfg<kM>::kSmem);
+    cudaError_t e = cudaFuncSetAttribute(dlinear_wgmma_kernel<kM, kCl>, cudaFuncAttributeMaxDynamicSharedMemorySize,
+                                         DlCfg<kM, kCl>::kSmem);
     if (e != cudaSuccess) return set_error(U2_ERR_CUDA, "dlinear: cudaFuncSetAttribute: %s", cudaGetErrorString(e));
     int per_sm = 0;
-    e = cudaOccupancyMaxActiveBlocksPerMultiprocessor(&per_sm, dlinear_wgmma_kernel<kM>, kDlThreads, DlCfg<kM>::kSmem);
+    e = cudaOccupancyMaxActiveBlocksPerMultiprocessor(&per_sm, dlinear_wgmma_kernel<kM, kCl>, kDlThreads, DlCfg<kM, kCl>::kSmem);
     if (e != cudaSuccess || per_sm < 1)
       return set_error(U2_ERR_CUDA, "dlinear: kernel cannot be resident on an SM (%s, %d CTA/SM): set U2_MULTI_OP=0",
                        cudaGetErrorString(e), per_sm);
     configured = true;
   }
-  int grid = num_sms();
+  return U2_OK;
+}
+
+static int cluster_shape(int* n_clusters, int* cluster_size) {
+  static int nc = 0, cs = 0;
+  if (!nc) {
+    int rc = configure_kernel<64, true>();
+    if (rc) return rc;
+    const int sms = num_sms();
+    if (sms <= 0) return set_error(U2_ERR_CUDA, "dlinear: cannot query SM count");
+    for (int c = kDlClusterMax; c >= 2 && !nc; c /= 2) {
+      cudaLaunchConfig_t cfg = {};
+      cfg.gridDim = dim3((unsigned)(sms / c * c));
+      cfg.blockDim = dim3(kDlThreads);
+      cfg.dynamicSmemBytes = DlCfg<64, true>::kSmem;
+      cudaLaunchAttribute attr[1];
+      attr[0].id = cudaLaunchAttributeClusterDimension;
+      attr[0].val.clusterDim.x = (unsigned)c;
+      attr[0].val.clusterDim.y = 1;
+      attr[0].val.clusterDim.z = 1;
+      cfg.attrs = attr;
+      cfg.numAttrs = 1;
+      int n = 0;
+      cudaError_t e = cudaOccupancyMaxActiveClusters(&n, dlinear_wgmma_kernel<64, true>, &cfg);
+      if (e != cudaSuccess) {
+        (void)cudaGetLastError();
+        n = 0;
+      }
+      if (n > 0) {
+        nc = n;
+        cs = c;
+      }
+    }
+    if (!nc) return set_error(U2_ERR_UNSUPPORTED, "dlinear: no cluster of 2 or 4 CTAs can be resident (cluster schedule)");
+  }
+  *n_clusters = nc;
+  *cluster_size = cs;
+  return U2_OK;
+}
+
+template <int kM, bool kCl>
+static int launch_multi_t(DlinMulti& mp, int pdl, cudaStream_t stream) {
+  int rc = configure_kernel<kM, kCl>();
+  if (rc) return rc;
+  int grid = num_sms(), csize = 1;
   if (grid <= 0) return set_error(U2_ERR_CUDA, "dlinear: cannot query SM count");
-  if (mp.n_ops == 1) {
+  if (kCl) {
+    int nc = 0;
+    rc = cluster_shape(&nc, &csize);
+    if (rc) return rc;
+    grid = nc * csize;
+  } else if (mp.n_ops == 1) {
     const long long work = (kM == 64) ? mp.op[0].num_tiles : (long long)mp.op[0].num_tiles * mp.op[0].kblocks;
     if (work < grid) grid = (int)work;
   }
   cudaLaunchConfig_t cfg = {};
   cfg.gridDim = dim3((unsigned)grid);
   cfg.blockDim = dim3(kDlThreads);
-  cfg.dynamicSmemBytes = DlCfg<kM>::kSmem;
+  cfg.dynamicSmemBytes = DlCfg<kM, kCl>::kSmem;
   cfg.stream = stream;
-  cudaLaunchAttribute attr[1];
-  attr[0].id = cudaLaunchAttributeProgrammaticStreamSerialization;
-  attr[0].val.programmaticStreamSerializationAllowed = 1;
+  cudaLaunchAttribute attr[2];
+  int na = 0;
+  if (pdl) {
+    attr[na].id = cudaLaunchAttributeProgrammaticStreamSerialization;
+    attr[na].val.programmaticStreamSerializationAllowed = 1;
+    ++na;
+  }
+  if (kCl) {
+    attr[na].id = cudaLaunchAttributeClusterDimension;
+    attr[na].val.clusterDim.x = (unsigned)csize;
+    attr[na].val.clusterDim.y = 1;
+    attr[na].val.clusterDim.z = 1;
+    ++na;
+  }
   cfg.attrs = attr;
-  cfg.numAttrs = pdl ? 1 : 0;
-  cudaError_t e = cudaLaunchKernelEx(&cfg, dlinear_wgmma_kernel<kM>, mp);
+  cfg.numAttrs = na;
+  cudaError_t e = cudaLaunchKernelEx(&cfg, dlinear_wgmma_kernel<kM, kCl>, mp);
   if (e != cudaSuccess) return set_error(U2_ERR_CUDA, "dlinear launch: %s", cudaGetErrorString(e));
   return U2_OK;
 }
 
-static int launch_multi(DlinMulti& mp, int kM, int pdl, cudaStream_t stream) {
-  return kM == 64 ? launch_multi_t<64>(mp, pdl, stream) : launch_multi_t<128>(mp, pdl, stream);
-}
-
-static inline int tile_m_of(const u2_dlinear_desc* d) { return d->sched == U2_DLIN_TILES64 ? 64 : 128; }
-
+static int launch_multi(DlinMulti& mp, int sched, int pdl, cudaStream_t stream) {
+  switch (sched) {
+    case U2_DLIN_TILES64: return launch_multi_t<64, false>(mp, pdl, stream);
+    case U2_DLIN_CLUSTER64: return launch_multi_t<64, true>(mp, pdl, stream);
+    default: return launch_multi_t<128, false>(mp, pdl, stream);
+  }
+}
+
+static inline int tile_m_of(int sched) { return sched == U2_DLIN_STREAMK128 ? 128 : 64; }
+
+static inline bool sched_ok(int sched) {
+  return sched == U2_DLIN_STREAMK128 || sched == U2_DLIN_TILES64 || sched == U2_DLIN_CLUSTER64;
+}
+
+extern "C" U2_API int32_t u2_dlinear_clusters(int32_t* cluster_size) {
+  int nc = 0, cs = 0;
+  if (cluster_shape(&nc, &cs)) return -1;
+  if (cluster_size) *cluster_size = cs;
+  return nc;
+}
 
 extern "C" U2_API int64_t u2_dlinear_ws_elems(int32_t N, int32_t K) {
   if (N <= 0 || K <= 0) return 0;
@@ -718,7 +942,8 @@
   static DlinMulti mp;
   mp.n_ops = 1;
   if (!d) return set_error(U2_ERR_ARG, "dlinear: null descriptor");
-  const int kM = tile_m_of(d);
+  if (!sched_ok(d->sched)) return set_error(U2_ERR_ARG, "dlinear: unknown schedule %d", d->sched);
+  const int kM = tile_m_of(d->sched);
   int rc = fill_op(x, w, y, d, &mp.op[0], &mp.tw[0], &mp.tx[0], kM);
   if (rc) return rc;
   mp.gridbar = nullptr;
@@ -727,7 +952,7 @@
   mp.pre_stages = 0;
   mp.dbg = reinterpret_cast<unsigned long long*>(d->dbg);
   mp.step_dev = d->counters;
-  return launch_multi(mp, kM, d->pdl, reinterpret_cast<cudaStream_t>(stream));
+  return launch_multi(mp, d->sched, d->pdl, reinterpret_cast<cudaStream_t>(stream));
 }
 
 extern "C" U2_API int u2_dlinear_multi_bf16(const void* const* x, const void* const* w, void* const* y,
@@ -739,9 +964,11 @@
   if (n_ops > 1 && (!gridbar || !step_dev)) return set_error(U2_ERR_ARG, "dlinear_multi: gridbar / step_dev required");
   static DlinMulti mp;
   mp.n_ops = n_ops;
-  const int kM = tile_m_of(&descs[0]);
+  const int sched = descs[0].sched;
+  if (!sched_ok(sched)) return set_error(U2_ERR_ARG, "dlinear_multi: unknown schedule %d", sched);
+  const int kM = tile_m_of(sched);
   for (int i = 0; i < n_ops; ++i) {
-    if (tile_m_of(&descs[i]) != kM) return set_error(U2_ERR_ARG, "dlinear_multi: all ops of a launch must share one schedule");
+    if (descs[i].sched != sched) return set_error(U2_ERR_ARG, "dlinear_multi: all ops of a launch must share one schedule");
     int rc = fill_op(x[i], w[i], y[i], &descs[i], &mp.op[i], &mp.tw[i], &mp.tx[i], kM);
     if (rc) return rc;
   }
@@ -762,7 +989,7 @@
   }
   mp.dbg = reinterpret_cast<unsigned long long*>(descs[0].dbg);
   mp.step_dev = step_dev ? step_dev : descs[0].counters;
-  return launch_multi(mp, kM, pdl, reinterpret_cast<cudaStream_t>(stream));
+  return launch_multi(mp, sched, pdl, reinterpret_cast<cudaStream_t>(stream));
 }
 
 extern "C" U2_API int u2_decode_embed_bf16(const int64_t* ids, const void* table, const float* gamma, void* x,
diff --git a/u2tokenizer_b200/csrc/ptx.cuh b/u2tokenizer_b200/csrc/ptx.cuh
--- a/u2tokenizer_b200/csrc/ptx.cuh
+++ b/u2tokenizer_b200/csrc/ptx.cuh
@@ -50,6 +50,64 @@
 __device__ __forceinline__ void mbar_wait(uint64_t* bar, uint32_t parity) {
   while (!mbar_try_wait(bar, parity)) {
   }
+}
+
+__device__ __forceinline__ uint32_t cluster_ctarank() {
+  uint32_t r;
+  asm volatile("mov.u32 %0, %%cluster_ctarank;" : "=r"(r));
+  return r;
+}
+
+__device__ __forceinline__ uint32_t cluster_nctarank() {
+  uint32_t r;
+  asm volatile("mov.u32 %0, %%cluster_nctarank;" : "=r"(r));
+  return r;
+}
+
+__device__ __forceinline__ uint32_t cluster_id_x() {
+  uint32_t r;
+  asm volatile("mov.u32 %0, %%clusterid.x;" : "=r"(r));
+  return r;
+}
+
+__device__ __forceinline__ uint32_t cluster_count_x() {
+  uint32_t r;
+  asm volatile("mov.u32 %0, %%nclusterid.x;" : "=r"(r));
+  return r;
+}
+
+__device__ __forceinline__ void cluster_sync_all() {
+  asm volatile("barrier.cluster.arrive.release;\n\tbarrier.cluster.wait.acquire;" ::: "memory");
+}
+
+__device__ __forceinline__ uint32_t mapa_shared(uint32_t addr, uint32_t rank) {
+  uint32_t r;
+  asm volatile("mapa.shared::cluster.u32 %0, %1, %2;" : "=r"(r) : "r"(addr), "r"(rank));
+  return r;
+}
+
+__device__ __forceinline__ void st_async_f4(uint32_t remote_addr, float a, float b, float c, float d, uint32_t remote_bar) {
+  asm volatile("st.async.shared::cluster.mbarrier::complete_tx::bytes.v4.f32 [%0], {%1, %2, %3, %4}, [%5];"
+               ::"r"(remote_addr), "f"(a), "f"(b), "f"(c), "f"(d), "r"(remote_bar)
+               : "memory");
+}
+
+__device__ __forceinline__ void mbar_arrive_remote(uint32_t remote_bar) {
+  asm volatile("mbarrier.arrive.release.cluster.shared::cluster.b64 _, [%0];" ::"r"(remote_bar) : "memory");
+}
+
+__device__ __forceinline__ bool mbar_try_wait_cluster(uint64_t* bar, uint32_t parity) {
+  uint32_t ok;
+  asm volatile(
+      "{\n\t"
+      ".reg .pred p;\n\t"
+      "mbarrier.try_wait.parity.acquire.cluster.shared::cta.b64 p, [%1], %2;\n\t"
+      "selp.u32 %0, 1, 0, p;\n\t"
+      "}"
+      : "=r"(ok)
+      : "r"(smem_u32(bar)), "r"(parity)
+      : "memory");
+  return ok != 0;
 }
 
 __device__ __forceinline__ void tma_prefetch_desc(const CUtensorMap* m) {
diff --git a/u2tokenizer_b200/engine.py b/u2tokenizer_b200/engine.py
--- a/u2tokenizer_b200/engine.py
+++ b/u2tokenizer_b200/engine.py
@@ -101,7 +101,7 @@
         self.fused_patch_embed = os.environ.get("U2_FUSED_PATCH_EMBED", "0") != "0"
         self.use_flash = os.environ.get("U2_FLASH", "1") != "0"
         self.fine_deps = os.environ.get("U2_FINE_DEPS", "0") != "0"
-        self.dl_sched = int(os.environ.get("U2_DL_SCHED", "0"))
+        self.dl_sched = int(os.environ.get("U2_DL_SCHED", str(ops.SCHED_STREAMK128)))
         self.pre_stages = int(os.environ.get("U2_PRE_STAGES", "0"))
         self.l2_lookahead_units = int(os.environ.get("U2_L2_LOOKAHEAD", "0"))
         self.l2_next_units = int(os.environ.get("U2_L2_NEXT", "-1"))
diff --git a/u2tokenizer_b200/ops.py b/u2tokenizer_b200/ops.py
--- a/u2tokenizer_b200/ops.py
+++ b/u2tokenizer_b200/ops.py
@@ -13,6 +13,7 @@
 
 ACT_NONE, ACT_GELU, ACT_SILU = 0, 1, 2
 DT_BF16, DT_F32 = 0, 1
+SCHED_STREAMK128, SCHED_TILES64, SCHED_CLUSTER64 = 0, 1, 2
 
 
 def _stream() -> int:
@@ -402,6 +403,14 @@
     return d
 
 
+def dlinear_clusters():
+    cs = C.c_int32(0)
+    n = int(_lib.load().u2_dlinear_clusters(C.byref(cs)))
+    if n < 0:
+        _lib.check(n, "u2_dlinear_clusters")
+    return n, int(cs.value)
+
+
 def dlinear_ws_elems(N: int, K: int) -> int:
     return int(_lib.load().u2_dlinear_ws_elems(N, K))
 
```

Result: no change. 2.141, median of 6 (+0.4%).
